# bluemoon-o2/walker-gym

Hardware: AMD Instinct MI355X
Metric: env-steps/sec (whole node) at 65 536 walkers; 1/2/4/8 MI355X scaling (higher is better)
Workload: dtype f32

## Files before the change

include/walker_hip.h:

```cpp
#ifndef WALKER_HIP_H
#define WALKER_HIP_H
#include <stdint.h>

#ifdef __cplusplus
extern "C" {
#endif

typedef struct ihipStream_t *hipStream_t;
typedef struct ihipEvent_t *hipEvent_t;

#define WG_ABI_VERSION 14
#define WG_EINVAL (-1)
#define WG_ERANGE (-2)
#define WG_EHIP (-3)

typedef struct wg_params {
    double g, dampk, ground, groundk, grounddamp, friction, dt;
    double pk, vk, ak, mk;
    int32_t in3d, max_steps;
    int32_t midform;
    int32_t conmid;
    int32_t spring_mode;
    int32_t action_mode;
    int32_t integrator;
    int32_t pair_mode;
    double pair_g;
    double pair_k;
    double pair_e;
    double bounce_k;
    double g3_gravity[3];
    double g3_damping;
    double g3_air;
    double g3_ground_level;
    double g3_restitution;
    double g3_friction;
    int32_t g3_ground;
    int32_t friction_mode;
} wg_params;

typedef struct wg_edge {
    uint32_t ij;
    float rest, k, c;
} wg_edge;

typedef struct wg_batch {
    int32_t N, M, K, A;
    int32_t ragged;
    const int32_t *mass_off, *edge_off, *muscle_off;
    float *pos, *vel, *acc;
    const float *mass;
    const wg_edge *edges;
    const uint16_t *inc;
    const uint16_t *inc_off;
    float *muscle_x;
    const float *muscle_bounds;
    const float *muscle_stride;
    int32_t *steps;
    uint8_t *contact;
    const uint8_t *pinned;
    const double *charge;
    double *radius;
    const int32_t *row;
    const uint8_t *bounce_set;
} wg_batch;

typedef struct wg_outputs {
    float *obs;       int32_t obs_stride;
    float *reward;    uint8_t *done;
    float *centroid;  float *energy;
    int64_t obs_step, out_step;
    int32_t obs_pad_clean;
    int32_t *steps;
    uint8_t *nonfinite;
    float *momentum;
} wg_outputs;

typedef struct wg_launch_info {
    int32_t threads, walkers_per_block, blocks, lds_bytes;
} wg_launch_info;

int wg_abi_version(void);
const char *wg_last_error(void);

int wg_step(const wg_batch *b, const wg_params *p, const float *action, int32_t action_cols,
            int32_t action_stride, int64_t action_step, const wg_outputs *o, int32_t n_steps,
            const int32_t *plan, int32_t plan_blocks, hipStream_t stream);

int wg_rollout(const wg_batch *b, const wg_params *p, const float *action, int32_t action_cols,
               int32_t action_stride, int64_t action_step, const wg_outputs *o, int32_t n_steps,
               const int32_t *plan, int32_t plan_blocks, hipStream_t stream);

typedef struct wg_range {
    const wg_batch *batch;
    const wg_outputs *outputs;
    int64_t action_offset;
    const int32_t *plan;
    int32_t plan_blocks;
    hipStream_t stream;
} wg_range;

int wg_step_ranges(const wg_range *ranges, int32_t n, const wg_params *p, const float *action, int32_t action_cols,
                   int32_t action_stride, hipEvent_t *events);

int wg_run_ranges(const wg_range *ranges, int32_t n, const wg_params *p, const float *action, int32_t action_cols,
                  int32_t action_stride, int64_t action_step, int32_t n_steps, hipEvent_t *events);

int wg_observe(const wg_batch *b, const wg_params *p, const wg_outputs *o, const int32_t *plan,
               int32_t plan_blocks, hipStream_t stream);

typedef wg_params wg_obs_cfg;
int wg_step_simple(const wg_batch *b, const float *action, const wg_params *p, int32_t n_steps, hipStream_t stream);
int wg_observe_simple(const wg_batch *b, const wg_obs_cfg *cfg, float *obs, float *reward, uint8_t *done,
                      float *centroid, float *energy, hipStream_t stream);

int wg_reset(const wg_batch *b, const wg_params *p, const float *noise, const uint8_t *mask,
             hipStream_t stream);

int wg_reset_noise(const wg_batch *b, const float *noise, hipStream_t stream);

int wg_plan_ragged(const int32_t *mass_off, const int32_t *edge_off, const int32_t *muscle_off,
                   int32_t N, int32_t *plan, int32_t max_blocks);

int wg_plan_waves(const int32_t *mass_off, const int32_t *edge_off, const int32_t *muscle_off,
                  int32_t N, int32_t *plan, int32_t max_tiles);
int wg_wave_edge_passes(int32_t M, int32_t K);

int wg_plan_errors(int32_t clear);

int wg_launch_geometry(const wg_batch *b, wg_launch_info *info);

int wg_debug_stamps(unsigned long long *host, int n);

int wg_launch_floor(int32_t mode, int32_t blocks, int32_t threads, const float *in, float *out, int32_t n_launches,
                    hipStream_t stream);

int wg_time_step(const wg_batch *batch, const wg_params *params, const float *action, int32_t action_cols,
                 int32_t action_stride, int64_t action_step, const wg_outputs *out, int32_t n_steps,
                 const int32_t *plan, int32_t plan_blocks, hipStream_t stream, float *ms_per_launch);

#ifdef __cplusplus
}
#endif
#endif
```

walker_gym_amd/_lib.py:

```python
from __future__ import annotations

import ctypes as C
import os
import threading

HERE = os.path.dirname(os.path.abspath(__file__))
LIB_NAME = "libwalker_hip.so"
LIB_PATH = os.path.join(HERE, LIB_NAME)
ABI_VERSION = 14

WG_EINVAL, WG_ERANGE, WG_EHIP = -1, -2, -3

_vp = C.c_void_p


class WgParams(C.Structure):
    _fields_ = [(n, C.c_double) for n in ("g", "dampk", "ground", "groundk", "grounddamp", "friction", "dt",
                                           "pk", "vk", "ak", "mk")] + \
               [(n, C.c_int32) for n in ("in3d", "max_steps", "midform", "conmid", "spring_mode", "action_mode",
                                         "integrator", "pair_mode")] + \
               [(n, C.c_double) for n in ("pair_g", "pair_k", "pair_e", "bounce_k")] + \
               [("g3_gravity", C.c_double * 3)] + \
               [(n, C.c_double) for n in ("g3_damping", "g3_air", "g3_ground_level", "g3_restitution",
                                          "g3_friction")] + [("g3_ground", C.c_int32), ("friction_mode", C.c_int32)]


class WgBatch(C.Structure):
    _fields_ = [("N", C.c_int32), ("M", C.c_int32), ("K", C.c_int32), ("A", C.c_int32),
                ("ragged", C.c_int32),
                ("mass_off", _vp), ("edge_off", _vp), ("muscle_off", _vp),
                ("pos", _vp), ("vel", _vp), ("acc", _vp), ("mass", _vp),
                ("edges", _vp),
                ("inc", _vp), ("inc_off", _vp),
                ("muscle_x", _vp), ("muscle_bounds", _vp), ("muscle_stride", _vp),
                ("steps", _vp), ("contact", _vp), ("pinned", _vp),
                ("charge", _vp), ("radius", _vp), ("row", _vp), ("bounce_set", _vp)]


class WgOutputs(C.Structure):
    _fields_ = [("obs", _vp), ("obs_stride", C.c_int32), ("reward", _vp), ("done", _vp),
                ("centroid", _vp), ("energy", _vp), ("obs_step", C.c_int64), ("out_step", C.c_int64),
                ("obs_pad_clean", C.c_int32), ("steps", _vp), ("nonfinite", _vp), ("momentum", _vp)]


class WgRange(C.Structure):
    _fields_ = [("batch", C.POINTER(WgBatch)), ("outputs", C.POINTER(WgOutputs)), ("action_offset", C.c_int64),
                ("plan", _vp), ("plan_blocks", C.c_int32), ("stream", _vp)]


class WgLaunchInfo(C.Structure):
    _fields_ = [("threads", C.c_int32), ("walkers_per_block", C.c_int32), ("blocks", C.c_int32),
                ("lds_bytes", C.c_int32)]


EXPORTS = ("wg_abi_version", "wg_last_error", "wg_step", "wg_step_ranges", "wg_run_ranges", "wg_rollout", "wg_observe",
           "wg_step_simple", "wg_observe_simple", "wg_reset", "wg_reset_noise", "wg_plan_ragged", "wg_plan_waves",
           "wg_wave_edge_passes", "wg_plan_errors", "wg_launch_geometry", "wg_launch_floor", "wg_time_step")

_lib = None
_lock = threading.Lock()


class WalkerHipError(RuntimeError):
    pass


def load(path: str | None = None):
    global _lib
    with _lock:
        if _lib is not None:
            return _lib
        p = path or os.environ.get("WALKER_HIP_LIB", LIB_PATH)
        if not os.path.exists(p):
            raise WalkerHipError(
                f"{p} not found: build it with `python -m walker_gym_amd.build` (hipcc --offload-arch=gfx950); "
                "walker_gym_amd has no CPU fallback")
        L = C.CDLL(p)
        L.wg_abi_version.restype = C.c_int
        L.wg_last_error.restype = C.c_char_p
        L.wg_step.argtypes = [C.POINTER(WgBatch), C.POINTER(WgParams), _vp, C.c_int32, C.c_int32, C.c_int64,
                              C.POINTER(WgOutputs), C.c_int32, _vp, C.c_int32, _vp]
        L.wg_rollout.argtypes = L.wg_step.argtypes
        L.wg_step_ranges.argtypes = [C.POINTER(WgRange), C.c_int32, C.POINTER(WgParams), _vp, C.c_int32, C.c_int32,
                                     C.POINTER(_vp)]
        L.wg_run_ranges.argtypes = [C.POINTER(WgRange), C.c_int32, C.POINTER(WgParams), _vp, C.c_int32, C.c_int32,
                                    C.c_int64, C.c_int32, C.POINTER(_vp)]
        L.wg_observe.argtypes = [C.POINTER(WgBatch), C.POINTER(WgParams), C.POINTER(WgOutputs), _vp, C.c_int32, _vp]
        L.wg_step_simple.argtypes = [C.POINTER(WgBatch), _vp, C.POINTER(WgParams), C.c_int32, _vp]
        L.wg_observe_simple.argtypes = [C.POINTER(WgBatch), C.POINTER(WgParams), _vp, _vp, _vp, _vp, _vp, _vp]
        L.wg_reset.argtypes = [C.POINTER(WgBatch), C.POINTER(WgParams), _vp, _vp, _vp]
        L.wg_reset_noise.argtypes = [C.POINTER(WgBatch), _vp, _vp]
        L.wg_plan_ragged.argtypes = [_vp, _vp, _vp, C.c_int32, _vp, C.c_int32]
        L.wg_plan_waves.argtypes = [_vp, _vp, _vp, C.c_int32, _vp, C.c_int32]
        L.wg_wave_edge_passes.argtypes = [C.c_int32, C.c_int32]
        L.wg_plan_errors.argtypes = [C.c_int32]
        L.wg_launch_geometry.argtypes = [C.POINTER(WgBatch), C.POINTER(WgLaunchInfo)]
        L.wg_launch_floor.argtypes = [C.c_int32, C.c_int32, C.c_int32, _vp, _vp, C.c_int32, _vp]
        L.wg_time_step.argtypes = L.wg_step.argtypes + [C.POINTER(C.c_float)]
        for f in EXPORTS[2:]:
            getattr(L, f).restype = C.c_int
        v = L.wg_abi_version()
        if v != ABI_VERSION:
            raise WalkerHipError(f"{p}: ABI version {v}, expected {ABI_VERSION}")
        _lib = L
        return L


def check(rc: int, what: str) -> int:
    if rc < 0:
        msg = load().wg_last_error().decode(errors="replace")
        exc = ValueError if rc in (WG_EINVAL, WG_ERANGE) else WalkerHipError
        raise exc(f"{what}: {msg} (code {rc})")
    return rc
```

walker_gym_amd/csrc/walker_hip.hip:

```cpp

#include <hip/hip_runtime.h>
#include <hip/hip_ext.h>

#include <algorithm>
#include <cstdarg>
#include <cstdint>
#include <cstdio>
#include <cstdlib>
#include <cstring>
#include <vector>

#include "walker_hip.h"
#include "powf2.h"

namespace {

thread_local char g_err[512] = "";

int fail(int code, const char *fmt, ...) __attribute__((format(printf, 2, 3)));
int fail(int code, const char *fmt, ...) {
    va_list ap;
    va_start(ap, fmt);
    vsnprintf(g_err, sizeof g_err, fmt, ap);
    va_end(ap);
    return code;
}

constexpr int WG_MAX_M = 1024;
constexpr double CONFIG_R = 16e-36;
constexpr int EPL = 4;
constexpr int NTHREADS = 256;
constexpr int MAXT = 512;
#ifndef WG_ABLATE
#define WG_ABLATE 0
#endif

struct KParams {
    float neg_g, neg_dampk, ground, neg_groundk, neg_grounddamp, friction, dt;
    float pk, vk, ak, mk, done_y;
    float dt2;
    double g;
    int max_steps, midform, conmid, spring_mode, action_mode;
    int integrator;
    int pair_mode;
    double pair_g, pair_k, pair_e;
    float bounce_kh;
    float g3g[3], g3_damp, g3_dragc, g3_level, g3_rest, g3_fric;
    int g3_ground;
    int friction_mode;
    int prio;
    int xcd;
};

struct KOut {
    float *obs, *reward;
    uint8_t *done;
    float *centroid, *energy;
    int32_t *steps;
    int64_t obs_step, out_step;
    int32_t obs_stride, obs_pad_clean;
};
inline KOut kout(const wg_outputs &o) {
    return KOut{o.obs, o.reward, o.done, o.centroid, o.energy, o.steps, o.obs_step, o.out_step, o.obs_stride,
                o.obs_pad_clean};
}

thread_local hipEvent_t g_kev_start = nullptr, g_kev_stop = nullptr;
#define WG_KLAUNCH(KERNEL, GRID, BLOCK, LDS, STREAM, ...)                                                          \
    do {                                                                                                          \
        if (g_kev_start)                                                                                          \
            hipExtLaunchKernelGGL(KERNEL, GRID, BLOCK, LDS, STREAM, g_kev_start, g_kev_stop, 0u, __VA_ARGS__);    \
        else                                                                                                      \
            hipLaunchKernelGGL(KERNEL, GRID, BLOCK, LDS, STREAM, __VA_ARGS__);                                    \
    } while (0)

__device__ __forceinline__ int xcd_block(int bid, int nwg) {
    const int q = nwg >> 3, r = nwg & 7, x = bid & 7;
    return (x < r ? x * (q + 1) : r * (q + 1) + (x - r) * q) + (bid >> 3);
}

struct Geo {
    int W, Pcap, Ecap, Ucap;
    int threads;
    int lds;
    float invM, invK, invA;
    int tbytes;
    int lite;
};

#ifdef WG_STAMPS
__device__ unsigned long long g_stamps[(1 << 16) * 8];
#define STAMP(k)                                                                                          \
    do {                                                                                                  \
        const unsigned long long t_ = __builtin_amdgcn_s_memtime();                                      \
        if ((threadIdx.x & 63) == 0 && stamp_wave < (1 << 16)) g_stamps[stamp_wave * 8 + (k)] = t_;      \
    } while (0)
#else
#define STAMP(k) do {} while (0)
#endif

struct Carve {
    double *t;
    float *pos, *vel, *acc, *m;
    float *df;
    uint32_t *inc;
    float *x;
    float *nrm, *ke, *pe;
    float *red;
    int *moff, *eoff, *uoff;
};

__host__ __device__ inline int align16(int b) { return (b + 15) & ~15; }

__device__ __forceinline__ int caller_row(const wg_batch &b, int w) { return b.row ? b.row[w] : w; }

enum { CV_T, CV_POS, CV_VEL, CV_ACC, CV_M, CV_DF, CV_INC, CV_X, CV_NRM, CV_KE, CV_PE, CV_RED,
       CV_MOFF, CV_EOFF, CV_UOFF, CV_N };
__host__ __device__ inline int carve_walk(const Geo &g, int *off) {
    int b = 0, k = 0;
    auto take = [&](int bytes) { off[k++] = b; b += align16(bytes); };
    const int full = g.lite ? 0 : 1;
    take(g.tbytes); take(g.Pcap * 12); take(g.Pcap * 12);
    take(full * g.Pcap * 12); take(full * g.Pcap * 4);
    take(g.Ecap * 12);
    take(g.Ecap * 4 + 16); take(g.Ucap * 4);
    take(full * g.Pcap * 4); take(full * g.Pcap * 4); take(full * g.Pcap * 4);
    take(full * g.W * 32);
    take(full * (g.W + 1) * 4); take(full * (g.W + 1) * 4); take(full * (g.W + 1) * 4);
    return b;
}
__host__ __device__ inline int carve_bytes(const Geo &g) { int off[CV_N]; return carve_walk(g, off); }
__device__ inline Carve carve(char *s, const Geo &g) {
    int o[CV_N];
    carve_walk(g, o);
    Carve c;
    c.t = reinterpret_cast<double *>(s + o[CV_T]); c.pos = reinterpret_cast<float *>(s + o[CV_POS]);
    c.vel = reinterpret_cast<float *>(s + o[CV_VEL]); c.acc = reinterpret_cast<float *>(s + o[CV_ACC]);
    c.m = reinterpret_cast<float *>(s + o[CV_M]); c.df = reinterpret_cast<float *>(s + o[CV_DF]);
    c.inc = reinterpret_cast<uint32_t *>(s + o[CV_INC]); c.x = reinterpret_cast<float *>(s + o[CV_X]);
    c.nrm = reinterpret_cast<float *>(s + o[CV_NRM]); c.ke = reinterpret_cast<float *>(s + o[CV_KE]);
    c.pe = reinterpret_cast<float *>(s + o[CV_PE]); c.red = reinterpret_cast<float *>(s + o[CV_RED]);
    c.moff = reinterpret_cast<int *>(s + o[CV_MOFF]); c.eoff = reinterpret_cast<int *>(s + o[CV_EOFF]);
    c.uoff = reinterpret_cast<int *>(s + o[CV_UOFF]);
    return c;
}

__device__ __forceinline__ float sqrt_mid(float s) {
    const float r = __builtin_amdgcn_sqrtf(s);
    const float rd = __uint_as_float(__float_as_uint(r) - 1u), ru = __uint_as_float(__float_as_uint(r) + 1u);
    float o = (__builtin_fmaf(-rd, r, s) <= 0.f) ? rd : r;
    return (__builtin_fmaf(-ru, r, s) > 0.f) ? ru : o;
}
__device__ inline float np_norm3(float x, float y, float z) {
    const float px = x * x, py = y * y, pz = z * z;
    double s = 0.0;
    s += (double)px; s += (double)py; s += (double)pz;
    return sqrtf((float)s);
}
__device__ inline float np_dot3(float ax, float ay, float az, float bx, float by, float bz) {
    const float p0 = ax * bx, p1 = ay * by, p2 = az * bz;
    double s = 0.0;
    s += (double)p0; s += (double)p1; s += (double)p2;
    return (float)s;
}
__device__ inline float seq_sum_lds(float r, const float *a, int n, int st) {
    int i = 0;
    for (; i + 4 <= n; i += 4) {
        const float x0 = a[i * st], x1 = a[(i + 1) * st], x2 = a[(i + 2) * st], x3 = a[(i + 3) * st];
        r = (((r + x0) + x1) + x2) + x3;
    }
    for (; i < n; i++) r += a[i * st];
    return r;
}
__device__ inline float pw_leaf(const float *a, int n, int st) {
    if (n < 8) return seq_sum_lds(0.f, a, n, st);
    float r0 = a[0], r1 = a[st], r2 = a[2 * st], r3 = a[3 * st];
    float r4 = a[4 * st], r5 = a[5 * st], r6 = a[6 * st], r7 = a[7 * st];
    int i = 8;
    for (; i < n - (n % 8); i += 8) {
        const float *p = a + i * st;
        r0 += p[0]; r1 += p[st]; r2 += p[2 * st]; r3 += p[3 * st];
        r4 += p[4 * st]; r5 += p[5 * st]; r6 += p[6 * st]; r7 += p[7 * st];
    }
    const float res = ((r0 + r1) + (r2 + r3)) + ((r4 + r5) + (r6 + r7));
    return seq_sum_lds(res, a + i * st, n - i, st);
}
__device__ inline void dual_sum_lds(const float *a, int sa, const float *p, int sp, int n, float &rs, float &rp) {
    float s = 0.f;
    int i = 0;
    if (n < 8) {
        float q = 0.f;
        for (; i + 4 <= n; i += 4) {
            const float x0 = a[i * sa], x1 = a[(i + 1) * sa], x2 = a[(i + 2) * sa], x3 = a[(i + 3) * sa];
            const float y0 = p[i * sp], y1 = p[(i + 1) * sp], y2 = p[(i + 2) * sp], y3 = p[(i + 3) * sp];
            s = (((s + x0) + x1) + x2) + x3;
            q = (((q + y0) + y1) + y2) + y3;
        }
        for (; i < n; i++) { s += a[i * sa]; q += p[i * sp]; }
        rs = s; rp = q;
        return;
    }
    float r0 = p[0], r1 = p[sp], r2 = p[2 * sp], r3 = p[3 * sp];
    float r4 = p[4 * sp], r5 = p[5 * sp], r6 = p[6 * sp], r7 = p[7 * sp];
    for (; i < 8; i += 4) {
        const float x0 = a[i * sa], x1 = a[(i + 1) * sa], x2 = a[(i + 2) * sa], x3 = a[(i + 3) * sa];
        s = (((s + x0) + x1) + x2) + x3;
    }
    for (; i < n - (n % 8); i += 8) {
        const float *q = p + i * sp, *b = a + i * sa;
        const float x0 = b[0], x1 = b[sa], x2 = b[2 * sa], x3 = b[3 * sa];
        const float x4 = b[4 * sa], x5 = b[5 * sa], x6 = b[6 * sa], x7 = b[7 * sa];
        r0 += q[0]; r1 += q[sp]; r2 += q[2 * sp]; r3 += q[3 * sp];
        r4 += q[4 * sp]; r5 += q[5 * sp]; r6 += q[6 * sp]; r7 += q[7 * sp];
        s = (((((((s + x0) + x1) + x2) + x3) + x4) + x5) + x6) + x7;
    }
    float res = ((r0 + r1) + (r2 + r3)) + ((r4 + r5) + (r6 + r7));
    for (; i < n; i++) { s += a[i * sa]; res += p[i * sp]; }
    rs = s; rp = res;
}
template <int D>
__device__ inline float pw_tree(const float *a, int n, int st) {
    if (D == 0 || n <= 128) return pw_leaf(a, n, st);
    int n2 = n / 2;
    n2 -= n2 % 8;
    return pw_tree<(D > 0 ? D - 1 : 0)>(a, n2, st) + pw_tree<(D > 0 ? D - 1 : 0)>(a + n2 * st, n - n2, st);
}
template <int PWD>
__device__ inline float np_pairwise(const float *a, int n, int st) { return pw_tree<PWD>(a, n, st); }

__device__ inline int locate(const int *off, int n, int x) {
    int lo = 0, hi = n - 1;
    while (lo < hi) {
        const int mid = (lo + hi + 1) >> 1;
        if (off[mid] <= x) lo = mid; else hi = mid - 1;
    }
    return lo;
}

__device__ inline int fdiv(int idx, int d, float inv) {
    (void)d;
    return (int)(((float)idx + 0.5f) * inv);
}

__device__ inline float fdiv_exact(float x, double y) { return (float)((double)x * y); }
constexpr int TINY_EXP = -79;
__device__ __forceinline__ int fexp(float x) { return __builtin_amdgcn_frexp_expf(x); }
__device__ __forceinline__ int fexp3(float a, float b, float c) { return min(min(fexp(a), fexp(b)), fexp(c)); }
__device__ __forceinline__ bool divisor_ok(float m) {
    const int e = fexp(m);
    return e >= -19 && e <= 21 && m != 0.f;
}
__device__ inline float fdiv_mk(float x, float m, float yf) {
    const float q = x * yf;
    if (!__builtin_isfinite(q) || yf == 0.f) return q;
    if (__builtin_expect(fexp(x) < TINY_EXP || !divisor_ok(m), 0)) return x / m;
    return __builtin_fmaf(__builtin_fmaf(-q, m, x), yf, q);
}
__device__ inline float fxsign(float v, uint32_t s) { return __uint_as_float(__float_as_uint(v) ^ s); }
__device__ inline double dxsign(double v, uint32_t s) {
    return __hiloint2double(__double2hiint(v) ^ (int)s, __double2loint(v));
}
__device__ inline double ddiv_fast(double a, double b, double y) {
    const double q = a * y;
    return __builtin_fma(__builtin_fma(-q, b, a), y, q);
}
__device__ inline float fdiv_fast(float x, float m, float yf) {
    const float q = x * yf;
    return __builtin_fmaf(__builtin_fmaf(-q, m, x), yf, q);
}
__device__ inline double ddiv_exact(double a, double b, double y) {
    const double q = a * y;
    if (!__builtin_isfinite(q) || y == 0.0) return q;
    return __builtin_fma(__builtin_fma(-q, b, a), y, q);
}
__device__ inline double ddiv_f32d(double a, double b, double y) {
    const double q = a * y;
    const double m = __builtin_fma(__builtin_fma(-q, b, a), y, q);
    const double am = __builtin_fabs(m);
    if (__builtin_expect(am >= 0x1p-800 && am <= 0x1p800, 1)) return m;
    return a == 0.0 ? q : a / b;
}

__device__ __forceinline__ double rcp64_nr(double d) {
    double y = __builtin_amdgcn_rcp(d);
    double e = __builtin_fma(-d, y, 1.0);
    y = __builtin_fma(y, e, y);
    e = __builtin_fma(-d, y, 1.0);
    return __builtin_fma(y, e, y);
}

__device__ __forceinline__ double rcp64_nr(double d);
__device__ __forceinline__ bool divisor_ok(float m);
__device__ __forceinline__ double recip_m(float mf) {
    const double md = (double)mf;
    double y = rcp64_nr(md);
    if (__builtin_expect(!divisor_ok(mf), 0)) y = 1.0 / md;
    return y;
}

__device__ __forceinline__ float fdiv_count(float x, float fM, double yM) {
    float q = (float)((double)x * yM);
    if (__builtin_expect(__builtin_fabsf(x) < 0x1p-100f, 0)) q = x / fM;
    return q;
}


__device__ __attribute__((noinline)) float np_sq_cold(float x) { return pw_pow2(x); }
template <bool INL = false>
__device__ __forceinline__ float np_sq(float x) {
    float f;
    if (__builtin_expect(!pw_pow2_fast(x, &f), 0)) f = INL ? pw_pow2(x) : np_sq_cold(x);
    return f;
}
__shared__ double s_pw_log2[32];
__shared__ unsigned long long s_pw_exp2[32];
__device__ __forceinline__ void pw_tables_to_lds(int tid) {
    if (tid < 32) { s_pw_log2[tid] = PW_LOG2_TAB[tid]; s_pw_exp2[tid] = PW_EXP2_TAB[tid]; }
}
__device__ __forceinline__ float pw_pow2_lds(float x) {
    unsigned int ix = pw_asu32(x) & 0x7fffffffu;
    if (ix == 0u || ix >= 0x7f800000u) return x * x;
    if (ix < 0x00800000u) {
        ix = pw_asu32(pw_asfloat(ix) * 0x1p23f) & 0x7fffffffu;
        ix -= 23u << 23;
    }
    const unsigned int tmp = ix - 0x3f330000u;
    const int i = (int)((tmp >> 19) & 15u);
    const unsigned int top = tmp & 0xff800000u;
    const int k = (int)top >> 23;
    const double invc = s_pw_log2[2 * i], logc = s_pw_log2[2 * i + 1];
    const double z = (double)pw_asfloat(ix - top);
    const double r = PW_FMA(z, invc, -1.0);
    const double y0 = logc + (double)k;
    const double r2 = r * r;
    double y = PW_FMA(0x1.27616c9496e0bp-2, r, -0x1.71969a075c67ap-2);
    const double p = PW_FMA(0x1.ec70a6ca7baddp-2, r, -0x1.7154748bef6c8p-1);
    const double r4 = r2 * r2;
    double q = PW_FMA(0x1.71547652ab82bp+0, r, y0);
    q = PW_FMA(p, r2, q);
    y = PW_FMA(y, r4, q);
    const double xd = 2.0 * y;
    if (((pw_asu64(xd) >> 47) & 0xffffu) >= (pw_asu64(126.0) >> 47)) {
        if (xd > 0x1.fffffffd1d571p+6) return pw_asfloat(0x7f800000u);
        if (xd <= -150.0) return 0.0f;
    }
    const double shift = 0x1.8p+47;
    double kd = xd + shift;
    const unsigned long long ki = pw_asu64(kd);
    kd -= shift;
    const double rr = xd - kd;
    const unsigned long long t = s_pw_exp2[ki & 31u] + (ki << 47);
    const double sc = pw_asdouble(t);
    const double zz = PW_FMA(0x1.c6af84b912394p-5, rr, 0x1.ebfce50fac4f3p-3);
    const double rr2 = rr * rr;
// ... 895 lines not shown
            if (pairs) {
                ax = s.acc[3 * lp]; ay = s.acc[3 * lp + 1]; az = s.acc[3 * lp + 2];
                mass_tail(kp, mf, (float)(1.0 / md), s.pos + 3 * lp, s.vel + 3 * lp, px, py, pz, vx, vy, vz, ax, ay,
                          az, hit, b.pinned && b.pinned[P0 + lp]);
            } else {
                mass_step(kp, s.t, s.df, s_inc16 + 2 * lb, lb, s0, (WG_ABLATE & 2) ? min(s1, s0 + 1) : s1, mf,
                          s.pos + 3 * lp, s.vel + 3 * lp, px, py, pz, vx, vy, vz, ax, ay, az, hit, kp.spring_mode,
                          b.pinned && b.pinned[P0 + lp], tiny_blk);
            }
            if (b.contact) b.contact[P0 + lp] = (uint8_t)hit;
            if (b.radius) b.radius[P0 + lp] = hit ? 3.0 : 1.0;
            s.pos[3 * lp] = px; s.pos[3 * lp + 1] = py; s.pos[3 * lp + 2] = pz;
            s.vel[3 * lp] = vx; s.vel[3 * lp + 1] = vy; s.vel[3 * lp + 2] = vz;
            if (SHFL) {
                float *ga = b.acc + 3 * ((size_t)P0 + lp);
                ga[0] = ax; ga[1] = ay; ga[2] = az;
            } else {
                s.acc[3 * lp] = ax; s.acc[3 * lp + 1] = ay; s.acc[3 * lp + 2] = az;
            }
            nv = np_norm3(vx, vy, vz);
            ke = mf * np_sq_t<true>(nv);
            pe = (float)(md * kp.g) * (py - kp.ground);
            if (!SHFL) { s.nrm[lp] = nv; s.ke[lp] = ke; s.pe[lp] = pe; }
        }
    } else {
        for (int lp = tid; lp < nP; lp += T) {
            const float mf = SHFL ? my_m : s.m[lp];
            vx = s.vel[3 * lp]; vy = s.vel[3 * lp + 1]; vz = s.vel[3 * lp + 2];
            px = s.pos[3 * lp]; py = s.pos[3 * lp + 1]; pz = s.pos[3 * lp + 2];
            if (SHFL) {
                const float *ga = b.acc + 3 * ((size_t)P0 + lp);
                ax = ga[0]; ay = ga[1]; az = ga[2];
            } else {
                ax = s.acc[3 * lp]; ay = s.acc[3 * lp + 1]; az = s.acc[3 * lp + 2];
            }
            nv = np_norm3(vx, vy, vz);
            ke = mf * np_sq_t<true>(nv);
            pe = (float)((double)mf * kp.g) * (py - kp.ground);
            if (!SHFL) { s.nrm[lp] = nv; s.ke[lp] = ke; s.pe[lp] = pe; }
        }
    }

    float midx = 0.f, midy = 0.f, midz = 0.f;
    float sumx = 0.f, sumy = 0.f, sumz = 0.f;
    const bool is_mass = tid < nP;
    const int my_q = tid - my_lm;
    if (SHFL) {
        const int M = b.M;
        const int gbase = (tid & ~63) + ((lane / M) * M);
        float sx, sy, sz;
        seq_sum3_lanes(px, py, pz, gbase, M, sx, sy, sz);
        const float ysum = pw_sum_lanes(py, gbase, M, lane), vsum = pw_sum_lanes(nv, gbase, M, lane);
        const float ksum = pw_sum_lanes(ke, gbase, M, lane), psum = pw_sum_lanes(pe, gbase, M, lane);
        const unsigned long long gmask = (M == 64) ? ~0ull : (((1ull << M) - 1ull) << (gbase & 63));
        const unsigned long long hb = __ballot(is_mass && (py - kp.ground < 0.f));
        const unsigned long long sb = __ballot(is_mass && nv < 0.1f);
        const int hits = __popcll(hb & gmask);
        const bool all_stopped = (sb & gmask) == gmask;
        const float fM = (float)M;
        midx = sx / fM; midy = sy / fM; midz = sz / fM;
        sumx = sx; sumy = sy; sumz = sz;
        if (is_mass && my_q == 0) {
            const size_t wg = (size_t)(w0 + my_wl);
            int steps = wsteps;
            if (STEP) { steps += 1; b.steps[wg] = steps; }
            if (o.steps) o.steps[wg] = steps;
            const float cy = ysum / fM;
            if (o.reward) {
                const float vpen = (-(vsum / fM)) * 0.1f;
                o.reward[wg] = (cy + vpen) + (float)(-(double)hits * 0.5);
            }
            if (o.done) {
                int done = steps >= kp.max_steps;
                if (!done && cy < kp.done_y) done = 1;
                if (!done && steps > 100) done = all_stopped;
                o.done[wg] = (uint8_t)done;
            }
            if (o.centroid) { o.centroid[3 * wg] = midx; o.centroid[3 * wg + 1] = midy; o.centroid[3 * wg + 2] = midz; }
            if (o.energy) o.energy[wg] = 0.5f * ksum + psum;
        }
    }
    __syncthreads();

    if (STEP) {
        stage_out(b.pos + 3 * (size_t)P0, s.pos, 3 * nP, tid, T);
        stage_out(b.vel + 3 * (size_t)P0, s.vel, 3 * nP, tid, T);
        if (!SHFL) stage_out(b.acc + 3 * (size_t)P0, s.acc, 3 * nP, tid, T);
    }
    if (!SHFL) {
        for (int idx = tid; idx < ((WG_ABLATE & 8) ? 0 : nw * 8); idx += T) {
            const int wl = idx >> 3, r = idx & 7;
            const int lm = RAGGED ? s.moff[wl] : wl * b.M;
            const int M = RAGGED ? s.moff[wl + 1] - lm : b.M;
            float v;
            if (r == 7) {
                int hits = 0, all = 1;
                for (int q = 0; q < M; q++) {
                    hits += (s.pos[3 * (lm + q) + 1] - kp.ground < 0.f);
                    all &= (s.nrm[lm + q] < 0.1f);
                }
                v = __int_as_float((hits << 1) | all);
            } else {
                const float *src = r < 3 ? s.pos + 3 * lm + r
                                 : r == 3 ? s.pos + 3 * lm + 1
                                 : r == 4 ? s.nrm + lm : r == 5 ? s.ke + lm : s.pe + lm;
                const int st = r <= 3 ? 3 : 1;
                if (r < 3) {
                    v = seq_sum_lds(0.f, src, M, st);
                } else {
                    v = np_pairwise<PWD>(src, M, st);
                }
            }
            s.red[idx] = v;
        }
        __syncthreads();
        if (tid < nw) {
            const int wl = tid;
            const int lm = RAGGED ? s.moff[wl] : wl * b.M;
            const int M = RAGGED ? s.moff[wl + 1] - lm : b.M;
            const size_t ws = (size_t)(w0 + wl);
            const size_t wg = (size_t)caller_row(b, w0 + wl);
            const float fM = (float)M;
            const float *rd = s.red + 8 * wl;
            const float cy = rd[3] / fM;
            const int packed = __float_as_int(rd[7]);
            const int hits = packed >> 1, all = packed & 1;
            int steps = wsteps;
            if (STEP) { steps += 1; b.steps[ws] = steps; }
            if (o.steps) o.steps[wg] = steps;
            if (o.reward) {
                const float av = rd[4] / fM;
                const float vpen = (-av) * 0.1f;
                const float cpen = (float)(-(double)hits * 0.5);
                o.reward[wg] = (cy + vpen) + cpen;
            }
            if (o.done) {
                int done = steps >= kp.max_steps;
                if (!done && cy < kp.done_y) done = 1;
                if (!done && steps > 100) done = all;
                o.done[wg] = (uint8_t)done;
            }
            if (o.centroid) {
                o.centroid[3 * wg] = rd[0] / fM; o.centroid[3 * wg + 1] = rd[1] / fM; o.centroid[3 * wg + 2] = rd[2] / fM;
            }
            if (o.energy) o.energy[wg] = 0.5f * rd[5] + rd[6];
        }
    }

    if (o.obs && !(WG_ABLATE & 16)) {
        constexpr int d = IN3D ? 3 : 2, per = 3 * d;
        const int stride = o.obs_stride;
        float *ob = o.obs + (uint32_t)w0 * (uint32_t)stride;
        float *tile = RAGGED ? nullptr : reinterpret_cast<float *>(s.t);
        const int nmid = kp.conmid ? 3 : 0;
        if (SHFL) {
            if (is_mass) {
                float *row = tile + (size_t)my_wl * stride + per * my_q;
                const float pm[3] = {px, py, pz}, vm[3] = {vx, vy, vz}, am[3] = {ax, ay, az};
                const float mm[3] = {kp.midform == 2 ? sumx : midx, kp.midform == 2 ? sumy : midy,
                                     kp.midform == 2 ? sumz : midz};
#pragma unroll
                for (int c = 0; c < d; c++) {
                    row[c] = kp.midform ? (pm[c] - mm[c]) * kp.pk : pm[c] * kp.pk;
                    row[d + c] = vm[c] * kp.vk;
                    row[2 * d + c] = am[c] * kp.ak;
                }
                if (my_q == 0 && nmid) {
                    float *wrow = tile + (size_t)my_wl * stride + per * b.M;
                    wrow[0] = kp.midform ? mm[0] : 0.f; wrow[1] = kp.midform ? mm[1] : 0.f; wrow[2] = kp.midform ? mm[2] : 0.f;
                }
                if (my_q == 0)
                    for (int r = per * b.M + nmid + b.A; r < stride; r++) tile[(size_t)my_wl * stride + r] = 0.f;
            }
        } else {
            for (int lp = tid; lp < nP; lp += T) {
                int wl, lm;
                if (lp == tid) { wl = my_wl; lm = my_lm; }
                else if (RAGGED) { wl = locate(s.moff, nw, lp); lm = s.moff[wl]; }
                else { wl = fdiv(lp, b.M, geo.invM); lm = wl * b.M; }
                const int M = RAGGED ? s.moff[wl + 1] - lm : b.M;
                const float fM = (float)M;
                float *row = (RAGGED ? o.obs + (size_t)caller_row(b, w0 + wl) * stride : tile + (size_t)wl * stride) +
                             per * (lp - lm);
#pragma unroll
                for (int c = 0; c < d; c++) {
                    const float pv = s.pos[3 * lp + c];
                    const float mid = kp.midform == 2 ? s.red[8 * wl + c] : s.red[8 * wl + c] / fM;
                    row[c] = kp.midform ? (pv - mid) * kp.pk : pv * kp.pk;
                    row[d + c] = s.vel[3 * lp + c] * kp.vk;
                    row[2 * d + c] = s.acc[3 * lp + c] * kp.ak;
                }
            }
            for (int wl = tid; wl < nw; wl += T) {
                const int lm = RAGGED ? s.moff[wl] : wl * b.M;
                const int M = RAGGED ? s.moff[wl + 1] - lm : b.M;
                const int A = RAGGED ? s.uoff[wl + 1] - s.uoff[wl] : b.A;
                float *row = RAGGED ? o.obs + (size_t)caller_row(b, w0 + wl) * stride : tile + (size_t)wl * stride;
                if (nmid)
                    for (int c = 0; c < 3; c++)
                        row[per * M + c] = kp.midform == 2 ? s.red[8 * wl + c] : kp.midform ? s.red[8 * wl + c] / (float)M : 0.f;
                for (int r = per * M + nmid + A; r < stride; r++) row[r] = 0.f;
            }
        }
        for (int u = tid; u < nU; u += T) {
            int wl, ua, M;
            if (RAGGED) { wl = locate(s.uoff, nw, u); ua = u - s.uoff[wl]; M = s.moff[wl + 1] - s.moff[wl]; }
            else { wl = fdiv(u, b.A, geo.invA); ua = u - wl * b.A; M = b.M; }
            (RAGGED ? o.obs + (size_t)caller_row(b, w0 + wl) * stride : tile + (size_t)wl * stride)[per * M + nmid + ua] =
                s.x[u] * kp.mk;
        }
        if (!RAGGED) {
            __syncthreads();
            stage_out(ob, tile, nw * stride, tid, T);
        }
    }
}


struct LeanGeo {
    int wpw;
    int wpb;
    int lgM;
    int slice;
    int off_df, off_inc, off_x;
    int pl;
    float invK, invA, invM;
    int nblk;
};

__device__ __forceinline__ void wave_sync() {
    __builtin_amdgcn_fence(__ATOMIC_RELEASE, "wavefront");
    __builtin_amdgcn_wave_barrier();
    __builtin_amdgcn_fence(__ATOMIC_ACQUIRE, "wavefront");
}


__device__ __forceinline__ float lane_gather(float v, int src_byte) {
    return __int_as_float(__builtin_amdgcn_ds_bpermute(src_byte, __float_as_int(v)));
}

__device__ __forceinline__ void spring_terms_cold(const EdgeRec &e, float x, float r0, float r1, float r2, double &t0,
                                               double &t1, double &t2, float &d0, float &d1, float &d2,
                                               int spring_mode) {
    const float cur = np_norm3(-r0, -r1, -r2);
    const float dx = cur - x;
    double dist = (double)cur;
    if (CONFIG_R > dist) dist = CONFIG_R;
    const float fsz = (spring_mode == 1 || !(dx < 0.f && edge_string(e.ij))) ? (-dx) * e.k : 0.f;
    const float nf = -fsz;
    d0 = r0; d1 = r1; d2 = r2;
    if (cur > 0.f) { d0 = r0 / cur; d1 = r1 / cur; d2 = r2 / cur; }
    if (spring_mode == 1) {
        t0 = (double)(fsz * d0); t1 = (double)(fsz * d1); t2 = (double)(fsz * d2);
    } else {
        t0 = (double)(nf * r0) / dist; t1 = (double)(nf * r1) / dist; t2 = (double)(nf * r2) / dist;
    }
}


__device__ __forceinline__ void spring_terms(const EdgeRec &e, float x, float pix, float piy, float piz, float pjx,
                                             float pjy, float pjz, float vix, float viy, float viz, float vjx,
                                             float vjy, float vjz, double &t0, double &t1, double &t2, float &g0,
                                             float &g1, float &g2, int spring_mode, bool pos_ok) {
    const float r0 = pjx - pix, r1 = pjy - piy, r2 = pjz - piz;
    float d0, d1, d2;
    const float sq = (float)(((double)(r0 * r0) + (double)(r1 * r1)) + (double)(r2 * r2));
    const bool mid = sq >= 0x1p-40f && sq < 0x1p40f;
    const float cur = sqrt_mid(sq);
    const float dx = cur - x;
    const double dist = (double)cur;
    const double yc = rcp64_nr(dist);
    const float fsz = (spring_mode == 1 || !(dx < 0.f && edge_string(e.ij))) ? (-dx) * e.k : 0.f;
    const float nf = -fsz;
    const float ycf = (float)yc;
    d0 = fdiv_fast(r0, cur, ycf); d1 = fdiv_fast(r1, cur, ycf); d2 = fdiv_fast(r2, cur, ycf);
    if (spring_mode == 1) {
        t0 = (double)(fsz * d0); t1 = (double)(fsz * d1); t2 = (double)(fsz * d2);
    } else {
        t0 = ddiv_fast((double)(nf * r0), dist, yc);
        t1 = ddiv_fast((double)(nf * r1), dist, yc);
        t2 = ddiv_fast((double)(nf * r2), dist, yc);
    }
    bool rok = true;
    if (__builtin_expect(!pos_ok, 0)) rok = fexp3(r0, r1, r2) >= TINY_EXP;
    const bool fast_ok = mid && rok && __builtin_fabsf(nf) < 0x1p100f;
    if (__builtin_expect(!fast_ok, 0)) spring_terms_cold(e, x, r0, r1, r2, t0, t1, t2, d0, d1, d2, spring_mode);
    const float dk = np_dot3(vix - vjx, viy - vjy, viz - vjz, d0, d1, d2);
    const float dkc = dk * e.c;
    g0 = dkc * d0; g1 = dkc * d1; g2 = dkc * d2;
}
template <class TS>
__device__ __forceinline__ void spring_edge_regs(const EdgeRec &e, int le, float x, float pix, float piy, float piz,
                                                 float pjx, float pjy, float pjz, float vix, float viy, float viz,
                                                 float vjx, float vjy, float vjz, const TS &ts, int spring_mode, bool &gt,
                                                 bool pos_ok) {
    double t0, t1, t2;
    float g0, g1, g2;
    spring_terms(e, x, pix, piy, piz, pjx, pjy, pjz, vix, viy, viz, vjx, vjy, vjz, t0, t1, t2, g0, g1, g2, spring_mode,
                 pos_ok);
    ts.put(le, t0, t1, t2, g0, g1, g2);
    gt = gt || fexp3(g0, g1, g2) < TINY_EXP;
}

template <int NE>
struct LeanIn {
    float p3[3], v3[3];
    EdgeRec er[NE];
    uint32_t gi[NE];
    float mf;
    int io0, io1, wsteps, pin;
    float x, lo, hi, stp, a;
};

struct LeanTile {
    int w0, nw, nP, nE, nU, wl, q, mu_wl, mu_ua;
    uint32_t P0, E0, U0;
    bool is_mass, is_mus, acts;
};

__device__ __forceinline__ LeanTile lean_tile_of(const wg_batch &b, const float *action, int action_cols,
                                                 const LeanGeo &lg, int tile, int lane) {
    LeanTile t;
    t.w0 = tile * lg.wpw;
    t.nw = min(lg.wpw, b.N - t.w0);
    t.nP = t.nw * b.M; t.nE = t.nw * b.K; t.nU = t.nw * b.A;
    t.P0 = (uint32_t)t.w0 * b.M; t.E0 = (uint32_t)t.w0 * b.K; t.U0 = (uint32_t)t.w0 * b.A;
    t.wl = lane >> lg.lgM; t.q = lane & (b.M - 1);
    t.is_mass = lane < t.nP;
    t.is_mus = lane < t.nU;
    t.mu_wl = b.A > 0 ? fdiv(lane, b.A, lg.invA) : 0;
    t.mu_ua = lane - t.mu_wl * b.A;
    t.acts = action != nullptr && t.is_mus && t.mu_ua < action_cols;
    return t;
}

template <typename T>
__device__ __forceinline__ const T &at_u32(const T *base, uint32_t byte_off) {
    return *reinterpret_cast<const T *>(reinterpret_cast<const char *>(base) + (size_t)byte_off);
}
template <typename T>
__device__ __forceinline__ T &at_u32w(T *base, uint32_t byte_off) {
    return *reinterpret_cast<T *>(reinterpret_cast<char *>(base) + (size_t)byte_off);
}
#define WG_ST(base, e, n) (&at_u32w((base), (uint32_t)(n) * 4u * (uint32_t)(e)))
__device__ __forceinline__ float neg_half_count(int n) { return -0.5f * (float)n; }
template <int NE>
__device__ __forceinline__ void lean_load_mass(const wg_batch &b, const LeanTile &t, int lane, LeanIn<NE> &L) {
    L.mf = 0.f; L.io0 = 0; L.io1 = 0; L.wsteps = 0; L.pin = 0;
    const int ln = min(lane, t.nP - 1);
    const int wl = ln >> (31 - __builtin_clz(b.M)), q = ln & (b.M - 1);
    L.mf = at_u32(b.mass, 4u * (t.P0 + ln));
    if (b.pinned) L.pin = at_u32(b.pinned, t.P0 + ln);
    const uint32_t io = (uint32_t)(t.w0 + wl) * (b.M + 1) + q;
    L.io0 = at_u32(b.inc_off, 2u * io); L.io1 = at_u32(b.inc_off, 2u * io + 2u);
    L.wsteps = at_u32(b.steps, 4u * (uint32_t)(t.w0 + wl));
}
template <int NE>
__device__ __forceinline__ void lean_load_muscles(const wg_batch &b, const KParams &kp, const float *__restrict__ action,
                                                  int action_stride, const LeanTile &t, int lane, LeanIn<NE> &L) {
    L.x = 0.f; L.lo = 0.f; L.hi = 0.f; L.stp = 0.f; L.a = 0.f;
    if (t.nU > 0) {
        const uint32_t ul = t.U0 + min(lane, t.nU - 1);
        L.x = at_u32(b.muscle_x, 4u * ul);
        if (action && action_stride > 0) {
            const float2 bd = at_u32(reinterpret_cast<const float2 *>(b.muscle_bounds), 8u * ul);
            L.lo = bd.x; L.hi = bd.y;
            if (kp.action_mode == 1) L.stp = at_u32(b.muscle_stride, 4u * ul);
            const int wl = min(t.mu_wl, t.nw - 1), ua = max(0, min(t.mu_ua, action_stride - 1));
            L.a = at_u32(action, 4u * ((uint32_t)(t.w0 + wl) * (uint32_t)action_stride + (uint32_t)ua));
        }
    }
}
template <int NE>
__device__ __forceinline__ void lean_load(const wg_batch &b, const KParams &kp, const float *__restrict__ action,
                                          int action_stride, const LeanTile &t, int lane, LeanIn<NE> &L) {
    const uint32_t pl = t.P0 + min(lane, t.nP - 1);
    const float *gp = &at_u32(b.pos, 12u * pl), *gv = &at_u32(b.vel, 12u * pl);
    L.p3[0] = gp[0]; L.p3[1] = gp[1]; L.p3[2] = gp[2];
    L.v3[0] = gv[0]; L.v3[1] = gv[1]; L.v3[2] = gv[2];
#pragma unroll
    for (int it = 0; it < NE; it++) {
        const uint32_t le = t.E0 + (uint32_t)min(lane + 64 * it, t.nE - 1);
        const uint4 v = at_u32(reinterpret_cast<const uint4 *>(b.edges), 16u * le);
        L.er[it] = EdgeRec{v.x, __uint_as_float(v.y), __uint_as_float(v.z), __uint_as_float(v.w)};
        L.gi[it] = at_u32(reinterpret_cast<const uint32_t *>(b.inc), 4u * le);
    }
    lean_load_mass<NE>(b, t, lane, L);
    lean_load_muscles<NE>(b, kp, action, action_stride, t, lane, L);
    if (!t.is_mass) {
        L.p3[0] = 0.f; L.p3[1] = 0.f; L.p3[2] = 0.f; L.v3[0] = 0.f; L.v3[1] = 0.f; L.v3[2] = 0.f;
        L.mf = 0.f; L.pin = 0; L.io0 = 0; L.io1 = 0;
    }
    if (!t.is_mus) { L.x = 0.f; L.lo = 0.f; L.hi = 0.f; L.stp = 0.f; }
    if (!t.acts) L.a = 0.f;
}

__device__ __forceinline__ double lane_gather_d(double v, int src_byte) {
    return __hiloint2double(__builtin_amdgcn_ds_bpermute(src_byte, __double2hiint(v)),
                            __builtin_amdgcn_ds_bpermute(src_byte, __double2loint(v)));
}

__device__ __forceinline__ float pw_pow2_lanes(float x, double tl, double te) {
    unsigned int ix = pw_asu32(x) & 0x7fffffffu;
    const bool special = ix == 0u || ix >= 0x7f800000u;
    if (ix < 0x00800000u && ix != 0u) {
        ix = pw_asu32(pw_asfloat(ix) * 0x1p23f) & 0x7fffffffu;
        ix -= 23u << 23;
    }
    const unsigned int tmp = ix - 0x3f330000u;
    const int i = (int)((tmp >> 19) & 15u);
    const unsigned int top = tmp & 0xff800000u;
    const int k = (int)top >> 23;
    const double invc = lane_gather_d(tl, (2 * i) << 2), logc = lane_gather_d(tl, (2 * i + 1) << 2);
    const double z = (double)pw_asfloat(ix - top);
    const double r = PW_FMA(z, invc, -1.0);
    const double y0 = logc + (double)k;
    const double r2 = r * r;
    double y = PW_FMA(0x1.27616c9496e0bp-2, r, -0x1.71969a075c67ap-2);
    const double p = PW_FMA(0x1.ec70a6ca7baddp-2, r, -0x1.7154748bef6c8p-1);
    const double r4 = r2 * r2;
    double q = PW_FMA(0x1.71547652ab82bp+0, r, y0);
    q = PW_FMA(p, r2, q);
    y = PW_FMA(y, r4, q);
    const double xd = 2.0 * y;
    const bool big = ((pw_asu64(xd) >> 47) & 0xffffu) >= (pw_asu64(126.0) >> 47);
    const double shift = 0x1.8p+47;
    double kd = xd + shift;
    const unsigned long long ki = pw_asu64(kd);
    kd -= shift;
    const double rr = xd - kd;
    const unsigned long long t = pw_asu64(lane_gather_d(te, (int)(ki & 31u) << 2)) + (ki << 47);
    const double sc = pw_asdouble(t);
    const double zz = PW_FMA(0x1.c6af84b912394p-5, rr, 0x1.ebfce50fac4f3p-3);
    const double rr2 = rr * rr;
    double yy = PW_FMA(0x1.62e42ff0c52d6p-1, rr, 1.0);
    yy = PW_FMA(zz, rr2, yy);
    float res = (float)(yy * sc);
    if (big && xd > 0x1.fffffffd1d571p+6) res = pw_asfloat(0x7f800000u);
    else if (big && xd <= -150.0) res = 0.0f;
    return special ? x * x : res;
}
__device__ __forceinline__ float np_sq_wave(float x, double tl, double te) {
    float f;
    const bool need = !pw_pow2_fast(x, &f);
    if (__builtin_expect(__ballot(need) != 0ull, 0)) {
        const float g = pw_pow2_lanes(x, tl, te);
        if (need) f = g;
    }
    return f;
}

__device__ __forceinline__ void pair_central(double coef, double sq, const float *p3, float mf, int lane, int M,
                                             bool is_mass, float &ax, float &ay, float &az, bool self_first = false) {
    const int gb = lane & ~(M - 1), q = lane & (M - 1);
    const double md = (double)mf, ym = 1.0 / md;
    const float sx = ax, sy = ay, sz = az;
    bool bad = false;
    {
        for (int pj = 0; pj < M; pj++) {
            const int src = (gb + pj) << 2;
            const float ox = lane_gather(p3[0], src), oy = lane_gather(p3[1], src), oz = lane_gather(p3[2], src);
            const double os = lane_gather_d(sq, src);
            if (!is_mass || pj == q) continue;
            const float d0 = ox - p3[0], d1 = oy - p3[1], d2 = oz - p3[2];
            const bool lo = pj < q && !self_first;
            pair_central_fast(coef, lo ? os : sq, lo ? sq : os, d0, d1, d2, md, ym, ax, ay, az, bad);
        }
        bad = is_mass && (bad || !__builtin_isfinite(ax + ay + az));
    }
    if (__builtin_expect(__ballot(bad) != 0, 0)) {
        float cx = sx, cy = sy, cz = sz;
        for (int pj = 0; pj < M; pj++) {
            const int src = (gb + pj) << 2;
            const float ox = lane_gather(p3[0], src), oy = lane_gather(p3[1], src), oz = lane_gather(p3[2], src);
            const double os = lane_gather_d(sq, src);
            if (!bad || pj == q) continue;
            const float d0 = ox - p3[0], d1 = oy - p3[1], d2 = oz - p3[2];
            const bool lo = pj < q && !self_first;
            pair_central_term(coef, lo ? os : sq, lo ? sq : os, d0, d1, d2, md, ym, cx, cy, cz);
        }
        if (bad) { ax = cx; ay = cy; az = cz; }
    }
}

__device__ __forceinline__ void pair_bounce(float kh, double rs, int bs, const float *p3, float mf, int lane, int M,
                                            bool is_mass, float &ax, float &ay, float &az) {
    const int gb = lane & ~(M - 1), q = lane & (M - 1);
    const double md = (double)mf, ym = 1.0 / md;
    for (int ph = 0; ph < 3; ph++) {
        for (int pj = 0; pj < M; pj++) {
            const int src = (gb + pj) << 2;
            const float ox = lane_gather(p3[0], src), oy = lane_gather(p3[1], src), oz = lane_gather(p3[2], src);
            const double orad = lane_gather_d(rs, src);
            const int obs = __builtin_amdgcn_ds_bpermute(src, bs);
            const bool on = ph == 1 ? pj != q && (bs & 1) && (obs & 2)
                                    : (ph == 0 ? pj < q : pj > q) && (obs & 1) && (bs & 2);
            if (!is_mass || !on) continue;
            const float d0 = ox - p3[0], d1 = oy - p3[1], d2 = oz - p3[2];
            const float cur = np_norm3(d0, d1, d2);
            const double x = rs + orad;
            if (!((double)cur <= x)) continue;
            const float dx = cur - (float)x;
            const float nf = -((-dx) * kh);
            bounce_term(cur, nf, d0, d1, d2, md, ym, ax, ay, az);
        }
    }
}

__device__ __forceinline__ void pair_g2_gravity(double g, const float *p3, float mf, int lane, int M, bool is_mass,
                                                float &ax, float &ay, float &az) {
    const int gb = lane & ~(M - 1), q = lane & (M - 1);
    const double md = (double)mf, ym = 1.0 / md;
    ax = 0.f; ay = 0.f; az = 0.f;
    for (int pj = 0; pj < M; pj++) {
        const int src = (gb + pj) << 2;
        const float ox = lane_gather(p3[0], src), oy = lane_gather(p3[1], src), oz = lane_gather(p3[2], src);
        const float om = lane_gather(mf, src);
        if (!is_mass || pj == q) continue;
        const double mo = (double)om;
        g2_gravity_term(((-g) * (pj < q ? mo : md)) * (pj < q ? md : mo), ox - p3[0], oy - p3[1], oz - p3[2], mf, ym,
                        ax, ay, az);
    }
}

__device__ __forceinline__ void pair_forces(const wg_batch &b, const KParams &kp, const float *p3, float mf,
                                         uint32_t pl, int lane, int M, bool is_mass, float &ax, float &ay,
                                         float &az) {
    if (kp.pair_mode & 1) pair_central(kp.pair_g, (double)mf, p3, mf, lane, M, is_mass, ax, ay, az);
    if (kp.pair_mode & 2) {
        const double e = (b.charge && is_mass) ? b.charge[pl] : kp.pair_e;
        pair_central(kp.pair_k, e, p3, mf, lane, M, is_mass, ax, ay, az);
    }
    if (kp.pair_mode & 4) {
        const double rs = is_mass ? b.radius[pl] : 0.0;
        const int bs = b.bounce_set ? (is_mass ? (int)b.bounce_set[pl] : 0) : 3;
        pair_bounce(kp.bounce_kh, rs, bs, p3, mf, lane, M, is_mass, ax, ay, az);
    }
    if (kp.pair_mode & 8) pair_g2_gravity(kp.pair_g, p3, mf, lane, M, is_mass, ax, ay, az);
    if (kp.pair_mode & 16) {
        const double e = (b.charge && is_mass) ? b.charge[pl] : kp.pair_e;
        pair_central(kp.pair_k, e, p3, mf, lane, M, is_mass, ax, ay, az, true);
    }
}



typedef TermsAoS LeanTerms;
__device__ __forceinline__ LeanTerms lean_terms(char *sl, const LeanGeo &lg) {
    return TermsAoS{reinterpret_cast<double *>(sl), reinterpret_cast<float *>(sl + lg.off_df)};
}

template <bool IN3D, int NE, bool RES = false>
__device__ __forceinline__ void lean_compute(const wg_batch &b, const KParams &kp, const KOut &o,
                                             const LeanGeo &lg, char *sl, const LeanTile &t, int lane,
                                             LeanIn<NE> &L, bool last = true) {
    const bool store = !RES || last;
    const int M = b.M, K = b.K, A = b.A;
    const int w0 = t.w0, nE = t.nE;
    const int wl = t.wl, q = t.q, mu_wl = t.mu_wl, mu_ua = t.mu_ua;
    const bool is_mass = t.is_mass, is_mus = t.is_mus, acts = t.acts;
    const uint32_t pl = t.P0 + lane, ul = t.U0 + lane;
    const LeanTerms ts = lean_terms(sl, lg);
#ifdef WG_STAMPS
    const int stamp_wave = t.w0 / lg.wpw;
#endif
    uint32_t *s_inc = reinterpret_cast<uint32_t *>(sl + lg.off_inc);
    float *s_x = reinterpret_cast<float *>(sl + lg.off_x);
    const float mf = L.mf;
    const bool pin = L.pin != 0;
    double sq_tl = 0.0, sq_te = 0.0;
    if (NE == 1 && !RES) {
        sq_tl = PW_LOG2_TAB[lane & 31];
        sq_te = pw_asdouble(PW_EXP2_TAB[lane & 31]);
    }

    if (!RES) {
#pragma unroll
        for (int it = 0; it < NE; it++)
            if (lane + 64 * it < nE) s_inc[lane + 64 * it] = L.gi[it];
        if (lane == 0) s_inc[nE] = 0u;
    }
    float x = L.x;
    if (acts) {
        x = (kp.action_mode == 1) ? ((L.a != 0.f) ? x + L.stp : x - L.stp) : x + L.a;
        if (L.lo > x) x = L.lo;
        if (L.hi < x) x = L.hi;
        if (store) *WG_ST(b.muscle_x, ul, 1) = x;
    }
    if (is_mus) s_x[lane] = x;
    double ym = recip_m(mf);
    if (!RES) asm volatile("" : "+v"(ym));
    wave_sync();
    STAMP(2);

    bool dead = false;
    if ((!RES || NE == 1) && kp.pair_mode == 0) {
        const bool nanp = is_mass && (__builtin_isnan(L.p3[0]) || __builtin_isnan(L.p3[1]) || __builtin_isnan(L.p3[2]));
        if (__builtin_expect(__ballot(nanp) != 0ull, 0)) {
            const unsigned long long db = __ballot(nanp && !pin && L.io1 > L.io0);
            const unsigned long long gm = (M == 64) ? ~0ull : (((1ull << M) - 1ull) << (lane & ~(M - 1)));
            dead = is_mass && (db & gm) == gm;
            if (dead) {
                L.p3[0] = (float)q; L.p3[1] = 0.f; L.p3[2] = 0.f;
                L.v3[0] = 0.f; L.v3[1] = 0.f; L.v3[2] = 0.f;
            }
        }
    }

    bool gtiny = false;
    const bool pos_ok = __all(fexp3(L.p3[0], L.p3[1], L.p3[2]) >= -55);
    struct Gath { float v[12]; };
    auto gather = [&](int it, Gath &g) {
        const int le = lane + 64 * it;
        const int ewl = fdiv(le, K, lg.invK);
        const uint32_t ij = L.er[it].ij;
        const int bi = ((ewl << lg.lgM) + edge_i(ij)) << 2, bj = ((ewl << lg.lgM) + edge_j(ij)) << 2;
#pragma unroll
        for (int c = 0; c < 3; c++) {
            if (WG_ABLATE & 512) {
                g.v[c] = L.p3[c]; g.v[3 + c] = L.p3[c] + (float)(bj - bi); g.v[6 + c] = L.v3[c]; g.v[9 + c] = L.v3[c];
                continue;
            }
            g.v[c] = lane_gather(L.p3[c], bi); g.v[3 + c] = lane_gather(L.p3[c], bj);
            g.v[6 + c] = lane_gather(L.v3[c], bi); g.v[9 + c] = lane_gather(L.v3[c], bj);
        }
    };
    auto spring = [&](int it, const Gath &g) {
        const int le = lane + 64 * it;
        const EdgeRec e = L.er[it];
        const int ewl = fdiv(le, K, lg.invK), ew = le - (int)__umul24(ewl, K);
        const bool mus = le < nE && ew < A;
        const float xs = s_x[mus ? (int)__umul24(ewl, A) + ew : 0];
        const float xr = mus ? xs : e.rest;
        if (le < nE) {
            if (WG_ABLATE & 1) {
                ts.put(le, xr + g.v[0] + g.v[3] + g.v[6] + g.v[9], g.v[1] + g.v[4] + g.v[7] + g.v[10],
                       g.v[2] + g.v[5] + g.v[8] + g.v[11], e.k, e.c, 0.f);
            } else {
                spring_edge_regs(e, le, xr, g.v[0], g.v[1], g.v[2], g.v[3], g.v[4], g.v[5], g.v[6], g.v[7], g.v[8],
                                 g.v[9], g.v[10], g.v[11], ts, 0, gtiny, pos_ok);
            }
        }
    };
#pragma unroll
    for (int it = 0; it < NE; it++) {
        if (64 * it >= nE) continue;
        if ((WG_ABLATE & 4096) && it == NE - 1 && it > 0) {
            const int le = lane + 64 * it;
            if (le < nE) ts.put(le, 0.0, 0.0, 0.0, 0.f, 0.f, 0.f);
            continue;
        }
        Gath g;
        gather(it, g);
        spring(it, g);
    }
    wave_sync();
    const bool wave_tiny = __any(gtiny);
    STAMP(3);

    EnvTerms et{};
    if (!RES) et = env_terms(kp, mf, (float)ym, L.v3[0], L.v3[1], L.v3[2]);
    float px = 0.f, py = 0.f, pz = 0.f, vx = 0.f, vy = 0.f, vz = 0.f, ax = 0.f, ay = 0.f, az = 0.f;
    float nv = 0.f, ke = 0.f, pe = 0.f;
    bool hit = false;
    if (is_mass) {
        const int r1 = (WG_ABLATE & 2) ? min(L.io1, L.io0 + 1) : L.io1;
        const int lb = wl * K;
        if (!RES)
            mass_accumulate_v2(ts, reinterpret_cast<const uint16_t *>(s_inc) + 2 * lb, lb, L.io0, r1, mf, ym, ax, ay, az,
                               wave_tiny);
        else
            mass_accumulate<LeanTerms, !RES>(ts, reinterpret_cast<const uint16_t *>(s_inc) + 2 * lb, lb, L.io0, r1, mf,
                                             ax, ay, az, 0, wave_tiny);
    }
    if (!RES && kp.pair_mode) pair_forces(b, kp, L.p3, mf, pl, lane, M, is_mass, ax, ay, az);
    if (is_mass) {
        mass_tail(kp, mf, (float)ym, L.p3, L.v3, px, py, pz, vx, vy, vz, ax, ay, az, hit, pin,
                  !RES ? &et : nullptr);
        if (dead) {
            px = __builtin_nanf(""); py = px; pz = px; vx = px; vy = px; vz = px; ax = px; ay = px; az = px;
            hit = false;
        }
        if (b.radius && store) b.radius[pl] = hit ? 3.0 : 1.0;
        nv = np_norm3(vx, vy, vz);
        if (!(NE == 1 && !RES)) ke = dead ? nv : mf * np_sq<NE == 1>(nv);
        pe = (float)((double)mf * kp.g) * (py - kp.ground);
    }
    if (NE == 1 && !RES) {
        const float sq = np_sq_wave(dead ? 0.f : nv, sq_tl, sq_te);
        if (is_mass) ke = dead ? nv : mf * sq;
    }
    STAMP(4);

    const int gbase = lane & ~(M - 1);
    const WalkerSums ws = (WG_ABLATE & 4) ? WalkerSums{px, py, pz, py, nv, ke, pe}
                                          : walker_sums(px, py, pz, nv, ke, pe, gbase, M, lane);
    const float sx = ws.sx, sy = ws.sy, sz = ws.sz, ysum = ws.ysum, vsum = ws.vsum, ksum = ws.ksum, psum = ws.psum;
    const unsigned long long gmask = (M == 64) ? ~0ull : (((1ull << M) - 1ull) << gbase);
    const unsigned long long hb = __ballot(is_mass && (py - kp.ground < 0.f));
    const unsigned long long sb = __ballot(is_mass && nv < 0.1f);
    const float midx = sx * lg.invM, midy = sy * lg.invM, midz = sz * lg.invM;
    if (is_mass) {
        if (store) {
            float *gpo = WG_ST(b.pos, pl, 3), *gvo = WG_ST(b.vel, pl, 3), *gao = WG_ST(b.acc, pl, 3);
            gpo[0] = px; gpo[1] = py; gpo[2] = pz;
            gvo[0] = vx; gvo[1] = vy; gvo[2] = vz;
            gao[0] = ax; gao[1] = ay; gao[2] = az;
            if (b.contact) at_u32w(b.contact, pl) = (uint8_t)hit;
        }
        if (q == 0) {
            const uint32_t wg = (uint32_t)(w0 + wl);
            const int steps = L.wsteps + 1;
            if (store) *WG_ST(b.steps, wg, 1) = steps;
            if (RES) L.wsteps = steps;
            if (o.steps) *WG_ST(o.steps, wg, 1) = steps;
            const float cy = ysum * lg.invM;
            if (o.reward) {
                const float vpen = (-(vsum * lg.invM)) * 0.1f;
                *WG_ST(o.reward, wg, 1) = (cy + vpen) + neg_half_count((int)__popcll(hb & gmask));
            }
            if (o.done) {
                int done = steps >= kp.max_steps;
                if (!done && cy < kp.done_y) done = 1;
                if (!done && steps > 100) done = (sb & gmask) == gmask;
                at_u32w(o.done, wg) = (uint8_t)done;
            }
            if (o.centroid) {
                float *c = WG_ST(o.centroid, wg, 3);
                c[0] = midx; c[1] = midy; c[2] = midz;
            }
            if (o.energy) *WG_ST(o.energy, wg, 1) = 0.5f * ksum + psum;
        }
    }

    STAMP(5);
    if (o.obs && !(WG_ABLATE & 16)) {
        constexpr int d = IN3D ? 3 : 2, per = 3 * d;
        const int stride = o.obs_stride, nmid = kp.conmid ? 3 : 0;
        typedef float fvd __attribute__((ext_vector_type(d), aligned(4)));
        if (is_mass) {
            const uint32_t row0 = (uint32_t)(w0 + wl) * (uint32_t)stride;
            const float mm[3] = {kp.midform == 2 ? sx : midx, kp.midform == 2 ? sy : midy, kp.midform == 2 ? sz : midz};
            const float pm[3] = {px, py, pz}, vm[3] = {vx, vy, vz}, am[3] = {ax, ay, az};
            fvd vp, vv, va;
#pragma unroll
            for (int c = 0; c < d; c++) {
                vp[c] = kp.midform ? (pm[c] - mm[c]) * kp.pk : pm[c] * kp.pk;
                vv[c] = vm[c] * kp.vk;
                va[c] = am[c] * kp.ak;
            }
            float *dst = WG_ST(o.obs, row0 + per * q, 1);
            *reinterpret_cast<fvd *>(dst) = vp;
            *reinterpret_cast<fvd *>(dst + d) = vv;
            *reinterpret_cast<fvd *>(dst + 2 * d) = va;
            if (q == 0) {
                if (nmid) {
                    float *mrow = WG_ST(o.obs, row0 + per * M, 1);
                    mrow[0] = kp.midform ? mm[0] : 0.f; mrow[1] = kp.midform ? mm[1] : 0.f;
                    mrow[2] = kp.midform ? mm[2] : 0.f;
                }
                for (int r = per * M + nmid + A; r < stride; r++) *WG_ST(o.obs, row0 + r, 1) = 0.f;
            }
        }
        if (is_mus) *WG_ST(o.obs, (uint32_t)(w0 + mu_wl) * (uint32_t)stride + per * M + nmid + mu_ua, 1) = x * kp.mk;
    }
    if (RES) {
        L.p3[0] = px; L.p3[1] = py; L.p3[2] = pz;
        L.v3[0] = vx; L.v3[1] = vy; L.v3[2] = vz;
        L.x = x;
    }
    STAMP(6);
#ifdef WG_STAMPS
    if (lane == 0 && stamp_wave < (1 << 16)) {
        const unsigned hw = __builtin_amdgcn_s_getreg((31 << 11) | 4);
        const unsigned xcc = __builtin_amdgcn_s_getreg((31 << 11) | 20);
        g_stamps[stamp_wave * 8 + 7] = (unsigned long long)hw | ((unsigned long long)xcc << 32);
    }
#endif
}

constexpr int lean_waves(int NE) { return NE >= 8 ? 4 : 6; }

template <bool IN3D, int NE>
__global__ __launch_bounds__(256) __attribute__((amdgpu_waves_per_eu(lean_waves(NE)))) void walker_step_lean(
    wg_batch b, KParams kp, const float *__restrict__ action, int action_cols, int action_stride, KOut o,
    LeanGeo lg) {
    extern __shared__ __attribute__((aligned(16))) char smem[];
    const int lane = threadIdx.x & 63, wv = __builtin_amdgcn_readfirstlane(threadIdx.x >> 6);
    const int blk = (kp.xcd & 2) ? xcd_block(blockIdx.x, gridDim.x) : (int)blockIdx.x;
    const int tile = blk * lg.wpb + wv;
    if (tile * lg.wpw >= b.N) return;
#ifdef WG_STAMPS
    const int stamp_wave = tile;
#endif
    STAMP(0);
    const LeanTile t = lean_tile_of(b, action, action_cols, lg, tile, lane);
    LeanIn<NE> L;
    if (kp.prio) __builtin_amdgcn_s_setprio(2);
    lean_load<NE>(b, kp, action, action_stride, t, lane, L);
    if (kp.prio) __builtin_amdgcn_s_setprio(0);
    STAMP(1);
    lean_compute<IN3D, NE>(b, kp, o, lg, smem + wv * lg.slice, t, lane, L);
}

template <bool IN3D>
__global__ __launch_bounds__(256) __attribute__((amdgpu_waves_per_eu(lean_waves(1)))) void walker_step_lean1(
    float *pos, float *vel, const wg_edge *edges, const uint16_t *inc, int N, int M, int K, int wpw, int wpb, int nblkx,
    wg_batch b, KParams kp, const float *__restrict__ action, int action_cols, int action_stride, KOut o, LeanGeo lg) {
    extern __shared__ __attribute__((aligned(16))) char smem[];
    b.pos = pos; b.vel = vel; b.edges = edges; b.inc = inc; b.N = N; b.M = M; b.K = K;
    lg.nblk = nblkx & 0x3fffffff; lg.wpw = wpw; lg.wpb = wpb;
    kp.prio = (int)((unsigned)nblkx >> 31);
    const int lane = threadIdx.x & 63, wv = __builtin_amdgcn_readfirstlane(threadIdx.x >> 6);
    const int bid = blockIdx.x, xb = xcd_block(bid, lg.nblk);
    const int blk = (nblkx & 0x40000000) ? xb : bid;
    const int tile = blk * lg.wpb + wv;
    if (tile * lg.wpw >= b.N) return;
#ifdef WG_STAMPS
    const int stamp_wave = tile;
#endif
    STAMP(0);
    const LeanTile t = lean_tile_of(b, action, action_cols, lg, tile, lane);
    LeanIn<1> L;
    if (kp.prio) __builtin_amdgcn_s_setprio(2);
    lean_load<1>(b, kp, action, action_stride, t, lane, L);
    if (kp.prio) __builtin_amdgcn_s_setprio(0);
    STAMP(1);
    lean_compute<IN3D, 1>(b, kp, o, lg, smem + wv * lg.slice, t, lane, L);
}

template <bool IN3D, int NE>
__global__ __launch_bounds__(256) __attribute__((amdgpu_waves_per_eu(NE >= 8 ? 4 : 5))) void walker_rollout_lean(
    wg_batch b, KParams kp, const float *__restrict__ action, int action_cols, int action_stride, int64_t action_step,
    KOut o, int n_steps, LeanGeo lg) {
    extern __shared__ __attribute__((aligned(16))) char smem[];
    const int lane = threadIdx.x & 63, wv = __builtin_amdgcn_readfirstlane(threadIdx.x >> 6);
    const int tile = blockIdx.x * lg.wpb + wv;
    if (tile * lg.wpw >= b.N) return;
#ifdef WG_STAMPS
    const int stamp_wave = tile;
#endif
    const LeanTile t = lean_tile_of(b, action, action_cols, lg, tile, lane);
    LeanIn<NE> L;
    if (kp.prio) __builtin_amdgcn_s_setprio(2);
    lean_load<NE>(b, kp, action, action_stride, t, lane, L);
    if (kp.prio) __builtin_amdgcn_s_setprio(0);
    {
        uint32_t *s_inc = reinterpret_cast<uint32_t *>(smem + wv * lg.slice + lg.off_inc);
#pragma unroll
        for (int it = 0; it < NE; it++)
            if (lane + 64 * it < t.nE) s_inc[lane + 64 * it] = L.gi[it];
    }
#pragma clang loop unroll(disable)
    for (int s = 0; s < n_steps; s++) {
        int ln = lane;
        asm volatile("" : "+v"(ln));
        const LeanTile ts = lean_tile_of(b, action, action_cols, lg, tile, ln);
        float a_next = 0.f;
        if (ts.acts && s + 1 < n_steps)
            a_next = action[(size_t)(s + 1) * (size_t)action_step +
                            (size_t)(uint32_t)(ts.w0 + ts.mu_wl) * (uint32_t)action_stride + (uint32_t)ts.mu_ua];
        KOut os = o;
        if (os.obs) os.obs += (size_t)s * os.obs_step;
        if (os.reward) os.reward += (size_t)s * os.out_step;
        if (os.done) os.done += (size_t)s * os.out_step;
        if (os.energy) os.energy += (size_t)s * os.out_step;
        if (os.centroid) os.centroid += 3 * (size_t)s * os.out_step;
        if (os.steps) os.steps += (size_t)s * os.out_step;
        asm volatile("" : "+v"(L.mf), "+v"(L.io0), "+v"(L.io1), "+v"(L.lo), "+v"(L.hi), "+v"(L.stp));
#pragma unroll
        for (int it = 0; it < NE; it++) asm volatile("" : "+v"(L.er[it].ij), "+v"(L.er[it].rest), "+v"(L.er[it].k),
                                                     "+v"(L.er[it].c));
        lean_compute<IN3D, NE, true>(b, kp, os, lg, smem + wv * lg.slice, ts, ln, L, s == n_steps - 1);
        L.a = a_next;
        wave_sync();
    }
}

constexpr int RW_MAXW = 32;
__device__ int g_plan_error;

struct RagGeo {
    int wpb;
    int slice;
    int off_df, off_inc, off_x, off_wo;
};


template <bool IN3D, int NE>
__global__ __launch_bounds__(256) __attribute__((amdgpu_waves_per_eu(NE >= 8 ? 4 : NE >= 4 ? 5 : 6))) void walker_step_waves(
    wg_batch b, KParams kp, const float *__restrict__ action, int action_cols, int action_stride, KOut o,
    const int32_t *__restrict__ plan, int ntiles, RagGeo rg) {
    extern __shared__ __attribute__((aligned(16))) char smem[];
    const int lane = threadIdx.x & 63, wv = __builtin_amdgcn_readfirstlane(threadIdx.x >> 6);
    const int blk = (kp.xcd & 1) ? xcd_block(blockIdx.x, gridDim.x) : (int)blockIdx.x;
    const int tile = blk * rg.wpb + wv;
    if (tile >= ntiles) return;
#ifdef WG_STAMPS
    const int stamp_wave = tile;
#endif
    STAMP(0);
    char *sl = smem + wv * rg.slice;
    const TermsAoS ts{reinterpret_cast<double *>(sl), reinterpret_cast<float *>(sl + rg.off_df)};
    uint32_t *s_inc = reinterpret_cast<uint32_t *>(sl + rg.off_inc);
    float *s_x = reinterpret_cast<float *>(sl + rg.off_x);
    int *s_mo = reinterpret_cast<int *>(sl + rg.off_wo);
    int *s_eo = s_mo + (RW_MAXW + 1), *s_uo = s_eo + (RW_MAXW + 1), *s_row = s_uo + (RW_MAXW + 1);
    float *s_mid = reinterpret_cast<float *>(s_row + RW_MAXW);
    float *s_tp = reinterpret_cast<float *>(sl);
    float *s_tn = s_tp + 192, *s_tk = s_tn + 64, *s_te = s_tk + 64;
    float *s_red = reinterpret_cast<float *>(sl + rg.off_df);

    if (kp.prio) __builtin_amdgcn_s_setprio(2);
    const int w0 = plan[tile], w1 = plan[tile + 1], nw = w1 - w0;
    const int P0 = b.mass_off[w0], E0 = b.edge_off[w0], U0 = b.muscle_off[w0];
    const int nP = b.mass_off[w1] - P0, nE = b.edge_off[w1] - E0, nU = b.muscle_off[w1] - U0;
    if (nw < 1 || nw > RW_MAXW || nP < 1 || nP > 64 || nU > 64 || nE > 64 * NE) {
        if (lane == 0) atomicOr(&g_plan_error, 1);
        return;
    }
    const bool is_mass = lane < nP, is_mus = lane < nU;
    const int lw = min(lane, nw), lr = min(lane, nw - 1);
    int wmo = at_u32(b.mass_off, 4u * (w0 + lw)) - P0, weo = at_u32(b.edge_off, 4u * (w0 + lw)) - E0;
    int wuo = at_u32(b.muscle_off, 4u * (w0 + lw)) - U0;
    int wsteps = at_u32(b.steps, 4u * (w0 + lr));
    const int lp = P0 + min(lane, max(nP, 1) - 1);
    float p3[3], v3[3];
    {
        const float *gp = &at_u32(b.pos, 12u * lp), *gv = &at_u32(b.vel, 12u * lp);
        p3[0] = gp[0]; p3[1] = gp[1]; p3[2] = gp[2];
        v3[0] = gv[0]; v3[1] = gv[1]; v3[2] = gv[2];
    }
    float mf = at_u32(b.mass, 4u * lp);
    EdgeRec er[NE];
    uint32_t gi[NE];
    if (nE > 0) {
#pragma unroll
        for (int it = 0; it < NE; it++) {
            const uint32_t le = E0 + min(lane + 64 * it, nE - 1);
            const uint4 v = at_u32(reinterpret_cast<const uint4 *>(b.edges), 16u * le);
            er[it] = EdgeRec{v.x, __uint_as_float(v.y), __uint_as_float(v.z), __uint_as_float(v.w)};
            gi[it] = at_u32(reinterpret_cast<const uint32_t *>(b.inc), 4u * le);
        }
    }
    float mx = 0.f, mlo = 0.f, mhi = 0.f, mst = 0.f;
    if (nU > 0) {
        const uint32_t lu = U0 + min(lane, nU - 1);
        mx = at_u32(b.muscle_x, 4u * lu);
        if (action) {
            const float2 bd = at_u32(reinterpret_cast<const float2 *>(b.muscle_bounds), 8u * lu);
            mlo = bd.x; mhi = bd.y;
            if (kp.action_mode == 1) mst = at_u32(b.muscle_stride, 4u * lu);
        }
    }
    int wrow = w0 + lr, pin = 0;
    if (b.row && !(WG_ABLATE & 2048)) wrow = at_u32(b.row, 4u * (w0 + lr));
    if (b.pinned) pin = at_u32(b.pinned, (uint32_t)lp);
    if (lane <= nw) { s_mo[lane] = wmo; s_eo[lane] = weo; s_uo[lane] = wuo; }
    if (lane < nw) s_row[lane] = wrow;
    int mw = 0, uw = 0, eww[NE];
#pragma unroll
    for (int it = 0; it < NE; it++) eww[it] = 0;
    for (int w = 1; w < nw; w++) {
        const int so = __builtin_amdgcn_readlane(wmo, w), se = __builtin_amdgcn_readlane(weo, w);
        const int su = __builtin_amdgcn_readlane(wuo, w);
        mw += lane >= so;
        uw += lane >= su;
#pragma unroll
        for (int it = 0; it < NE; it++) eww[it] += lane + 64 * it >= se;
    }
    if (!is_mass) mw = 0;
    if (!is_mus) uw = 0;
    wave_sync();
    const int mlm = s_mo[mw], mlb = s_eo[mw];
    const uint32_t io = (uint32_t)lp + (uint32_t)(w0 + mw);
    int io0 = at_u32(b.inc_off, 2u * io), io1 = at_u32(b.inc_off, 2u * io + 2u);
    const int ua = lane - s_uo[uw];
    const bool acts = action != nullptr && is_mus && ua < action_cols;
    float act = 0.f;
    if (action && action_cols > 0)
        act = at_u32(action, 4u * ((uint32_t)s_row[uw] * (uint32_t)action_stride + (uint32_t)min(max(ua, 0), action_cols - 1)));
    if (!is_mass) {
        p3[0] = 0.f; p3[1] = 0.f; p3[2] = 0.f; v3[0] = 0.f; v3[1] = 0.f; v3[2] = 0.f;
        mf = 0.f; pin = 0; io0 = 0; io1 = 0;
    }
    if (!is_mus) { mx = 0.f; mlo = 0.f; mhi = 0.f; mst = 0.f; }
    if (!acts) act = 0.f;
    bool dead = false;
    {
        const bool nanp = is_mass && (__builtin_isnan(p3[0]) || __builtin_isnan(p3[1]) || __builtin_isnan(p3[2]));
        if (__builtin_expect(__ballot(nanp) != 0ull, 0)) {
            const unsigned long long db = __ballot(nanp && pin == 0 && io1 > io0);
            const int mwn = s_mo[mw + 1] - mlm;
            const unsigned long long gm = (mwn >= 64) ? ~0ull : (((1ull << mwn) - 1ull) << mlm);
            dead = is_mass && (db & gm) == gm;
            if (dead) {
                p3[0] = (float)(lane - mlm); p3[1] = 0.f; p3[2] = 0.f;
                v3[0] = 0.f; v3[1] = 0.f; v3[2] = 0.f;
            }
        }
    }
    if (kp.prio) __builtin_amdgcn_s_setprio(0);
    STAMP(1);

#pragma unroll
    for (int it = 0; it < NE; it++)
        if (lane + 64 * it < nE) s_inc[lane + 64 * it] = gi[it];
    if (lane == 0) s_inc[nE] = 0u;
    float x = mx;
    if (acts) {
        x = (kp.action_mode == 1) ? ((act != 0.f) ? x + mst : x - mst) : x + act;
        if (mlo > x) x = mlo;
        if (mhi < x) x = mhi;
        *WG_ST(b.muscle_x, U0 + lane, 1) = x;
    }
    if (is_mus) s_x[lane] = x;
    double ym = recip_m(mf);
    asm volatile("" : "+v"(ym));
    wave_sync();
    STAMP(2);

    bool gtiny = false;
    const bool pos_ok = __all(fexp3(p3[0], p3[1], p3[2]) >= -55);
#pragma unroll
    for (int it = 0; it < NE; it++) {
        if (64 * it >= nE) continue;
        const int le = lane + 64 * it;
        const EdgeRec e = er[it];
        const int ew_w = le < nE ? eww[it] : 0;
        const int elm = s_mo[ew_w], ew = le - s_eo[ew_w], eA = s_uo[ew_w + 1] - s_uo[ew_w];
        const int bi = (elm + edge_i(e.ij)) << 2, bj = (elm + edge_j(e.ij)) << 2;
        const float pix = lane_gather(p3[0], bi), piy = lane_gather(p3[1], bi), piz = lane_gather(p3[2], bi);
        const float pjx = lane_gather(p3[0], bj), pjy = lane_gather(p3[1], bj), pjz = lane_gather(p3[2], bj);
        const float vix = lane_gather(v3[0], bi), viy = lane_gather(v3[1], bi), viz = lane_gather(v3[2], bi);
        const float vjx = lane_gather(v3[0], bj), vjy = lane_gather(v3[1], bj), vjz = lane_gather(v3[2], bj);
        const bool mus = le < nE && ew < eA;
        const float xs = s_x[mus ? s_uo[ew_w] + ew : 0];
        const float xr = mus ? xs : e.rest;
        if (le < nE) {
            if (WG_ABLATE & 1)
                ts.put(le, xr + pix + pjx + vix + vjx, piy + pjy + viy + vjy, piz + pjz + viz + vjz, e.k, e.c, 0.f);
            else
                spring_edge_regs(e, le, xr, pix, piy, piz, pjx, pjy, pjz, vix, viy, viz, vjx, vjy, vjz, ts, 0, gtiny,
                                 pos_ok);
        }
    }
    wave_sync();
    const bool wave_tiny = __any(gtiny);
    STAMP(3);

    EnvTerms et{};
    et = env_terms(kp, mf, (float)ym, v3[0], v3[1], v3[2]);
    float px = 0.f, py = 0.f, pz = 0.f, vx = 0.f, vy = 0.f, vz = 0.f, ax = 0.f, ay = 0.f, az = 0.f;
    bool hit = false;
    if (is_mass) {
        mass_accumulate_v2(ts, reinterpret_cast<const uint16_t *>(s_inc) + 2 * mlb, mlb, io0,
                           (WG_ABLATE & 2) ? min(io1, io0 + 1) : io1, mf, ym, ax, ay, az, wave_tiny);
        mass_tail(kp, mf, (float)ym, p3, v3, px, py, pz, vx, vy, vz, ax, ay, az, hit, pin != 0, &et);
        if (dead) {
            px = __builtin_nanf(""); py = px; pz = px; vx = px; vy = px; vz = px; ax = px; ay = px; az = px;
            hit = false;
        }
        const uint32_t pl = (uint32_t)(P0 + lane);
        float *gpo = WG_ST(b.pos, pl, 3), *gvo = WG_ST(b.vel, pl, 3), *gao = WG_ST(b.acc, pl, 3);
        gpo[0] = px; gpo[1] = py; gpo[2] = pz;
        gvo[0] = vx; gvo[1] = vy; gvo[2] = vz;
        gao[0] = ax; gao[1] = ay; gao[2] = az;
        if (b.contact) at_u32w(b.contact, pl) = (uint8_t)hit;
        if (b.radius) b.radius[pl] = hit ? 3.0 : 1.0;
    }
    STAMP(4);
    const float nvm = is_mass ? np_norm3(vx, vy, vz) : 0.f;
    const unsigned long long hb = __ballot(is_mass && (py - kp.ground < 0.f));
    const unsigned long long sb = __ballot(is_mass && nvm < 0.1f);
    wave_sync();
    if (is_mass) {
        const float nv = nvm;
        s_tp[3 * lane] = px; s_tp[3 * lane + 1] = py; s_tp[3 * lane + 2] = pz;
        s_tn[lane] = nv;
        s_tk[lane] = dead ? nv : mf * np_sq(nv);
        s_te[lane] = (float)((double)mf * kp.g) * (py - kp.ground);
    }
    wave_sync();

    for (int idx = lane; idx < ((WG_ABLATE & 32) ? 0 : nw * 8); idx += 64) {
        const int w = idx >> 3, r = idx & 7;
        const int lm = s_mo[w], M = s_mo[w + 1] - lm;
        float v;
        if (r == 7) {
            const unsigned long long wm = (M == 64) ? ~0ull : (((1ull << M) - 1ull) << lm);
            v = __int_as_float((__popcll(hb & wm) << 1) | ((sb & wm) == wm ? 1 : 0));
        } else {
            const float *src = r == 3 ? s_tp + 3 * lm + 1 : r == 5 ? s_tk + lm : r == 6 ? s_te + lm : s_tn + lm;
            float vs, vp;
            dual_sum_lds(s_tp + 3 * lm + (r < 3 ? r : 0), 3, src, r == 3 ? 3 : 1, M, vs, vp);
            v = r < 3 ? vs : vp;
        }
        s_red[idx] = v;
    }
    wave_sync();
    if (lane < nw) {
        const int M = s_mo[lane + 1] - s_mo[lane];
        const float fM = (float)M;
        const double yM = rcp64_nr((double)M);
        const float *rd = s_red + 8 * lane;
        const float cy = fdiv_count(rd[3], fM, yM);
        const int packed = __float_as_int(rd[7]);
        const int hits = packed >> 1, all = packed & 1;
        const int steps = wsteps + 1;
        *WG_ST(b.steps, w0 + lane, 1) = steps;
        if (o.steps) *WG_ST(o.steps, wrow, 1) = steps;
        if (o.reward) *WG_ST(o.reward, wrow, 1) = (cy + (-fdiv_count(rd[4], fM, yM)) * 0.1f) + neg_half_count(hits);
        if (o.done) {
            int done = steps >= kp.max_steps;
            if (!done && cy < kp.done_y) done = 1;
            if (!done && steps > 100) done = all;
            at_u32w(o.done, (uint32_t)wrow) = (uint8_t)done;
        }
        const float mx = fdiv_count(rd[0], fM, yM), my = fdiv_count(rd[1], fM, yM), mz = fdiv_count(rd[2], fM, yM);
        s_mid[3 * lane] = mx; s_mid[3 * lane + 1] = my; s_mid[3 * lane + 2] = mz;
        if (o.centroid) {
            float *c = WG_ST(o.centroid, wrow, 3);
            c[0] = mx; c[1] = my; c[2] = mz;
        }
        if (o.energy) *WG_ST(o.energy, wrow, 1) = 0.5f * rd[5] + rd[6];
    }
    wave_sync();
    STAMP(5);

    if (o.obs && !(WG_ABLATE & 16)) {
        constexpr int d = IN3D ? 3 : 2, per = 3 * d;
        const int stride = o.obs_stride, nmid = kp.conmid ? 3 : 0;
        typedef float fvd __attribute__((ext_vector_type(d), aligned(4)));
        if (is_mass) {
            const float *rd = kp.midform == 2 ? s_red + 8 * mw : s_mid + 3 * mw;
            float *dst = WG_ST(o.obs, (uint32_t)s_row[mw] * (uint32_t)stride + per * (lane - mlm), 1);
            const float pm[3] = {px, py, pz}, vm[3] = {vx, vy, vz}, am[3] = {ax, ay, az};
            fvd vp, vv, va;
#pragma unroll
            for (int c = 0; c < d; c++) {
                const float mid = rd[c];
                vp[c] = kp.midform ? (pm[c] - mid) * kp.pk : pm[c] * kp.pk;
                vv[c] = vm[c] * kp.vk;
                va[c] = am[c] * kp.ak;
            }
            *reinterpret_cast<fvd *>(dst) = vp;
            *reinterpret_cast<fvd *>(dst + d) = vv;
            *reinterpret_cast<fvd *>(dst + 2 * d) = va;
        }
        if (lane < nw && nmid) {
            const int M = s_mo[lane + 1] - s_mo[lane];
            float *row = WG_ST(o.obs, (uint32_t)wrow * (uint32_t)stride + per * M, 1);
            const float *rd = s_red + 8 * lane;
            for (int c = 0; c < 3; c++) row[c] = kp.midform == 2 ? rd[c] : kp.midform ? rd[c] / (float)M : 0.f;
        }
        if (is_mus)
            *WG_ST(o.obs, (uint32_t)s_row[uw] * (uint32_t)stride + per * (s_mo[uw + 1] - s_mo[uw]) + nmid + ua, 1) =
                x * kp.mk;
        if (!o.obs_pad_clean) {
            const float inv = 1.f / (float)stride;
            for (int i = lane; i < nw * stride; i += 64) {
                const int w = fdiv(i, stride, inv), c = i - w * stride;
                const int len = per * (s_mo[w + 1] - s_mo[w]) + nmid + (s_uo[w + 1] - s_uo[w]);
                if (c >= len) *WG_ST(o.obs, (uint32_t)s_row[w] * (uint32_t)stride + c, 1) = 0.f;
            }
        }
    }
    STAMP(6);
#ifdef WG_STAMPS
    if (lane == 0 && stamp_wave < (1 << 16)) {
        const unsigned hw = __builtin_amdgcn_s_getreg((31 << 11) | 4);
        const unsigned xcc = __builtin_amdgcn_s_getreg((31 << 11) | 20);
        g_stamps[stamp_wave * 8 + 7] = (unsigned long long)hw | ((unsigned long long)xcc << 32);
    }
#endif
}

__global__ void walker_reset_kernel(wg_batch b, const float *__restrict__ noise, const uint8_t *__restrict__ mask,
                                    int zmode) {
    const int P = b.ragged ? b.mass_off[b.N] : b.N * b.M;
    for (int q = blockIdx.x * blockDim.x + threadIdx.x; q < P; q += gridDim.x * blockDim.x) {
        int w;
        if (b.ragged) {
            int lo = 0, hi = b.N - 1;
            while (lo < hi) { const int mid = (lo + hi + 1) >> 1; if (b.mass_off[mid] <= q) lo = mid; else hi = mid - 1; }
            w = lo;
        } else {
            w = q / b.M;
        }
        if (mask && !mask[w]) continue;
        if (noise) {
#pragma unroll
            for (int c = 0; c < 3; c++) {
                const float n = noise[3 * q + c];
                const bool add = zmode == 2 ? __float_as_uint(n) != 0u : (c < 2 || zmode == 1);
                if (add) b.vel[3 * q + c] = b.vel[3 * q + c] + n;
            }
        }
    }
    for (int w = blockIdx.x * blockDim.x + threadIdx.x; w < b.N; w += gridDim.x * blockDim.x)
        if (!mask || mask[w]) b.steps[w] = 0;
}

__global__ __launch_bounds__(256) void walker_info_kernel(wg_batch b, uint8_t *__restrict__ nonfinite,
                                                          float *__restrict__ momentum, const int32_t *__restrict__ plan,
                                                          int plan_blocks) {
    const int w = blockIdx.x * blockDim.x + threadIdx.x;
    if (w >= b.N) return;
    if (plan && (w < plan[0] || w >= plan[plan_blocks])) return;
    const int p0 = b.ragged ? b.mass_off[w] : w * b.M, p1 = b.ragged ? b.mass_off[w + 1] : p0 + b.M;
    float mx = 0.f, my = 0.f, mz = 0.f;
    bool bad = false;
    for (int q = p0; q < p1; q++) {
        const float *pv = b.pos + 3 * (size_t)q, *vv = b.vel + 3 * (size_t)q, *av = b.acc + 3 * (size_t)q;
        const float vx = vv[0], vy = vv[1], vz = vv[2], m = b.mass[q];
        bad = bad || !(__builtin_isfinite(pv[0]) && __builtin_isfinite(pv[1]) && __builtin_isfinite(pv[2]) &&
                       __builtin_isfinite(vx) && __builtin_isfinite(vy) && __builtin_isfinite(vz) &&
                       __builtin_isfinite(av[0]) && __builtin_isfinite(av[1]) && __builtin_isfinite(av[2]));
        mx = mx + vx * m; my = my + vy * m; mz = mz + vz * m;
    }
    const int r = caller_row(b, w);
    if (nonfinite) nonfinite[r] = (uint8_t)bad;
    if (momentum) { momentum[3 * r] = mx; momentum[3 * r + 1] = my; momentum[3 * r + 2] = mz; }
}

int env_int(const char *name, int dflt);
int wave_passes(int M, int K);

KParams make_kparams(const wg_params &p) {
    KParams k;
    k.neg_g = (float)(-p.g);
    k.neg_dampk = (float)(-p.dampk);
    k.ground = (float)p.ground;
    k.neg_groundk = (float)(-p.groundk);
    k.neg_grounddamp = (float)(-p.grounddamp);
    k.friction = (float)p.friction;
    k.dt = (float)p.dt;
    k.pk = (float)p.pk; k.vk = (float)p.vk; k.ak = (float)p.ak; k.mk = (float)p.mk;
    k.done_y = (float)(p.ground - 50.0);
    k.g = p.g;
    k.max_steps = p.max_steps; k.midform = p.midform; k.conmid = p.conmid;
    k.spring_mode = p.spring_mode; k.action_mode = p.action_mode;
    k.integrator = p.integrator;
    k.pair_mode = p.pair_mode;
    k.pair_g = p.pair_g;
    k.pair_k = p.pair_k;
    k.pair_e = p.pair_e;
    k.bounce_kh = (float)(p.bounce_k / 2);
    for (int i = 0; i < 3; i++) k.g3g[i] = (float)p.g3_gravity[i];
    k.g3_damp = (float)p.g3_damping;
    k.g3_dragc = (float)(-0.5 * p.g3_air);
    k.g3_level = (float)p.g3_ground_level;
    k.g3_rest = (float)p.g3_restitution;
    k.g3_fric = (float)p.g3_friction;
    k.g3_ground = p.g3_ground;
    k.friction_mode = p.friction_mode;
    k.prio = env_int("WG_LEAN_PRIO", 1);
    k.xcd = env_int("WG_XCD", 3);

    k.dt2 = (float)(p.dt * p.dt);
    return k;
}

constexpr int RAG_P = 256, RAG_E = 512, RAG_U = 256, RAG_W = 64;
constexpr int LDS_LIMIT = 160 * 1024;

int validate(const wg_batch *b) {
    if (!b) return fail(WG_EINVAL, "null batch");
    if (b->N < 0 || b->M < 1 || b->K < 0 || b->A < 0 || b->A > b->K)
        return fail(WG_EINVAL, "bad sizes N=%d M=%d K=%d A=%d", b->N, b->M, b->K, b->A);
    if (2 * b->K > 65535) return fail(WG_ERANGE, "K=%d exceeds the u16 incidence encoding", b->K);
    if (b->M > WG_MAX_M) return fail(WG_ERANGE, "M=%d > %d masses per walker", b->M, WG_MAX_M);
    if (!b->pos || !b->vel || !b->acc || !b->mass || !b->steps || !b->muscle_x)
        return fail(WG_EINVAL, "missing state pointer");
    if (b->K > 0 && (!b->edges || !b->inc || !b->inc_off)) return fail(WG_EINVAL, "missing edge pointer");
    if (b->M > 32767) return fail(WG_ERANGE, "M=%d exceeds the 15-bit edge endpoint encoding", b->M);
    if (!b->inc_off) return fail(WG_EINVAL, "missing inc_off");
    if (b->ragged < 0 || b->ragged > 2) return fail(WG_EINVAL, "ragged must be 0, 1 or 2");
    if (b->ragged && (!b->mass_off || !b->edge_off || !b->muscle_off))
        return fail(WG_EINVAL, "ragged batch without offsets");
    if (!b->ragged && b->row) return fail(WG_EINVAL, "row (a walker permutation) is for ragged batches only");
    if (b->ragged == 2 && !wave_passes(b->M, b->K))
        return fail(WG_EINVAL, "ragged = 2 (wave tiles) needs M <= 64 and at most 8 spring passes (M=%d K=%d)", b->M, b->K);
    return 0;
}

Geo uniform_geo(const wg_batch *b, int obs_stride, bool no_lite = false) {
    Geo g{};
    int W = std::max(1, NTHREADS / b->M);
    if (b->M > 64 && env_int("WG_WIDE", 1)) {
        int best = 0, bestT = NTHREADS;
        for (int T = NTHREADS; T <= MAXT; T += 64) {
            const int w = T / b->M;
            if (w >= 1 && (int64_t)w * b->M * bestT > (int64_t)best * T) { best = w * b->M; bestT = T; W = w; }
        }
    }
    if (b->K > 0) W = std::max(1, std::min(W, EPL * MAXT / std::max(1, b->K)));
    while (W > 1 && (b->N + W - 1) / W < 512) W = std::max(1, W / 2);
    g.W = W;
    const bool shfl_shape = b->M <= 64 && (64 % b->M) == 0 && !(WG_ABLATE & 64);
    for (;;) {
        g.Pcap = g.W * b->M; g.Ecap = g.W * b->K; g.Ucap = g.W * b->A;
        g.tbytes = std::max(g.Ecap * 3 * 8, g.W * std::max(0, obs_stride) * 4);
        g.lite = (shfl_shape && g.W * b->M <= MAXT && !no_lite) ? 1 : 0;
        g.threads = std::min(MAXT, std::max(64, ((g.W * b->M + 63) / 64) * 64));
        if (b->K > 0 && g.W * b->K > EPL * g.threads) g.threads = MAXT;
        g.lds = carve_bytes(g);
        if (g.lds <= 64 * 1024 || g.W == 1) break;
        g.W = std::max(1, g.W / 2);
    }
    g.invM = 1.f / (float)b->M;
    g.invK = 1.f / (float)std::max(1, b->K);
    g.invA = 1.f / (float)std::max(1, b->A);
    return g;
}

Geo ragged_geo(const wg_batch *b) {
    Geo g{};
    g.threads = NTHREADS;
    g.W = RAG_W;
    g.Pcap = std::max(RAG_P, b->M);
    g.Ecap = std::max(RAG_E, b->K);
    g.Ucap = std::max(RAG_U, b->A);
    g.tbytes = g.Ecap * 3 * 8;
    g.lite = 0;
    g.lds = carve_bytes(g);
    g.invM = g.invK = g.invA = 0.f;
    return g;
}

template <bool STEP, bool RAGGED, bool IN3D, int PWD, bool SHFL>
int launch(const wg_batch *b, const KParams &kp, const float *action, int cols, int astride,
           const wg_outputs &o, const int32_t *plan, int blocks, const Geo &g, hipStream_t stream) {
    const int lds_static = (int)(sizeof(s_pw_log2) + sizeof(s_pw_exp2));
    if (g.lds + lds_static > LDS_LIMIT)
        return fail(WG_ERANGE, "workgroup needs %d B of LDS (> 160 KiB)", g.lds + lds_static);
    WG_KLAUNCH((walker_step_kernel<STEP, RAGGED, IN3D, PWD, SHFL>), dim3(blocks), dim3(g.threads), (uint32_t)g.lds, stream,
               *b, kp, action, cols, astride, kout(o), plan, g);
    const hipError_t e = hipGetLastError();
    if (e != hipSuccess) return fail(WG_EHIP, "launch failed: %s", hipGetErrorString(e));
    return 0;
}

bool shfl_ok(const wg_batch *b, const Geo &g) { return !b->ragged && g.lite; }

template <bool STEP, int PWD>
int dispatch2(const wg_batch *b, const KParams &kp, bool in3d, const float *a, int cols, int astride,
              const wg_outputs &o, const int32_t *plan, int blocks, const Geo &g, hipStream_t st) {
    if (b->ragged) {
        return in3d ? launch<STEP, true, true, PWD, false>(b, kp, a, cols, astride, o, plan, blocks, g, st)
                    : launch<STEP, true, false, PWD, false>(b, kp, a, cols, astride, o, plan, blocks, g, st);
    }
    if (PWD == 0 && shfl_ok(b, g)) {
        return in3d ? launch<STEP, false, true, 0, true>(b, kp, a, cols, astride, o, plan, blocks, g, st)
                    : launch<STEP, false, false, 0, true>(b, kp, a, cols, astride, o, plan, blocks, g, st);
    }
    return in3d ? launch<STEP, false, true, PWD, false>(b, kp, a, cols, astride, o, plan, blocks, g, st)
                : launch<STEP, false, false, PWD, false>(b, kp, a, cols, astride, o, plan, blocks, g, st);
}
int env_int(const char *name, int dflt) {
    const char *e = getenv(name);
    return (e && *e) ? atoi(e) : dflt;
}

bool lean_enabled() { return env_int("WG_LEAN", 1) != 0; }

bool u32_bytes(const wg_batch *b) {
    const int64_t lim = 1ll << 32;
    return (int64_t)b->N * b->M * 12 < lim && (int64_t)b->N * b->K * 16 < lim && (int64_t)b->N * b->A * 8 < lim &&
           (int64_t)b->N * (b->M + 1) * 2 < lim;
}
bool obs_u32(const wg_batch *b, int obs_stride) { return (int64_t)b->N * std::max(obs_stride, 1) * 4 < (1ll << 32); }

bool lean_geo(const wg_batch *b, int obs_stride, LeanGeo *out, int spring_mode = 0) {
    const int M = b->M;
    if (b->ragged || M < 4 || M > 64 || (64 % M) != 0 || b->K < 1 || !lean_enabled() || (WG_ABLATE & 128)) return false;
    if (spring_mode != 0) return false;
    if ((int64_t)b->N * b->M * 3 >= (1ll << 31) || (int64_t)b->N * b->K * 4 >= (1ll << 31) ||
        !obs_u32(b, obs_stride) || !u32_bytes(b))
        return false;
    LeanGeo g{};
    g.wpw = 64 / M;
    while (g.wpw > 1 && (b->N + g.wpw - 1) / g.wpw < 512) g.wpw >>= 1;
    const int wcap = env_int("WG_LEAN_WPW", 0);
    if (wcap > 0 && wcap < g.wpw) g.wpw = wcap;
    g.lgM = 0;
    while ((1 << g.lgM) < M) g.lgM++;
    if ((g.wpw * b->K + 63) / 64 > 8 || g.wpw * b->A > 64) return false;
    const int wpb = env_int("WG_LEAN_WAVES", 0);
    g.wpb = (wpb == 1 || wpb == 2 || wpb == 4) ? wpb : ((b->N + g.wpw - 1) / g.wpw <= 1024 ? 1 : 4);
    const int ew = g.wpw * b->K;
    g.pl = (ew + 3) & ~3;
    g.off_df = align16(g.pl * 24);
    g.off_inc = g.off_df + align16(g.pl * 12);
    g.off_x = g.off_inc + align16(ew * 4 + 4);
    g.slice = g.off_x + align16(std::max(1, g.wpw * b->A) * 4);
    if (4 * g.slice > 80 * 1024) return false;
    g.invK = 1.f / (float)b->K;
    g.invA = 1.f / (float)std::max(1, b->A);
    g.invM = 1.f / (float)M;
    g.nblk = (b->N + g.wpb * g.wpw - 1) / (g.wpb * g.wpw);
    *out = g;
    return true;
}

int lean_blocks(const wg_batch *b, const LeanGeo &g) { return (b->N + g.wpb * g.wpw - 1) / (g.wpb * g.wpw); }

int launch_lean(const wg_batch *b, const KParams &kp, bool in3d, const float *a, int cols, int astride,
                const wg_outputs &o, const LeanGeo &g, hipStream_t st) {
    const int blocks = lean_blocks(b, g);
    const int ne = (g.wpw * b->K + 63) / 64;
    const int lds = g.wpb * g.slice + std::max(0, env_int("WG_LDS_PAD", 0));
#define WG_LAUNCH_LEAN(D3, NE_)                                                                                  \
    WG_KLAUNCH((walker_step_lean<D3, NE_>), dim3(blocks), dim3(64 * g.wpb), (uint32_t)lds, st, *b, kp, a, cols,  \
               astride, kout(o), g)
#define WG_LEAN_NE(D3)                                                         \
    do {                                                                       \
        if (ne == 2) WG_LAUNCH_LEAN(D3, 2);                                    \
        else if (ne == 3) WG_LAUNCH_LEAN(D3, 3);                               \
        else if (ne == 4) WG_LAUNCH_LEAN(D3, 4);                               \
        else WG_LAUNCH_LEAN(D3, 8);                                            \
    } while (0)
    if (ne <= 1) {
        if (in3d)
            WG_KLAUNCH((walker_step_lean1<true>), dim3(blocks), dim3(64 * g.wpb), (uint32_t)lds, st, b->pos, b->vel,
                               b->edges, b->inc, b->N, b->M, b->K, g.wpw, g.wpb, (int)((unsigned)g.nblk | ((unsigned)(kp.xcd & 2) << 29) | ((unsigned)(kp.prio != 0) << 31)), *b,
                               kp, a, cols, astride, kout(o), g);
        else
            WG_KLAUNCH((walker_step_lean1<false>), dim3(blocks), dim3(64 * g.wpb), (uint32_t)lds, st, b->pos, b->vel,
                               b->edges, b->inc, b->N, b->M, b->K, g.wpw, g.wpb, (int)((unsigned)g.nblk | ((unsigned)(kp.xcd & 2) << 29) | ((unsigned)(kp.prio != 0) << 31)), *b,
                               kp, a, cols, astride, kout(o), g);
    } else if (in3d) {
        WG_LEAN_NE(true);
    } else {
        WG_LEAN_NE(false);
    }
#undef WG_LEAN_NE
#undef WG_LAUNCH_LEAN
    const hipError_t e = hipGetLastError();
    if (e != hipSuccess) return fail(WG_EHIP, "launch failed: %s", hipGetErrorString(e));
    return 0;
}

int launch_lean_rollout(const wg_batch *b, const KParams &kp, bool in3d, const float *a, int cols, int astride,
                        int64_t astep, const wg_outputs &o, int n_steps, const LeanGeo &g, hipStream_t st) {
    const int blocks = lean_blocks(b, g);
    const int ne = (g.wpw * b->K + 63) / 64;
    const int lds = g.wpb * g.slice;
#define WG_LAUNCH_RO(D3, NE_)                                                                                    \
    hipLaunchKernelGGL((walker_rollout_lean<D3, NE_>), dim3(blocks), dim3(64 * g.wpb), lds, st, *b, kp, a, cols, \
                       astride, astep, kout(o), n_steps, g)
#define WG_RO_NE(D3)                                                                                             \
    do {                                                                                                         \
        if (ne <= 1) WG_LAUNCH_RO(D3, 1);                                                                        \
        else if (ne == 2) WG_LAUNCH_RO(D3, 2);                                                                   \
        else if (ne == 3) WG_LAUNCH_RO(D3, 3);                                                                   \
        else if (ne == 4) WG_LAUNCH_RO(D3, 4);                                                                   \
        else WG_LAUNCH_RO(D3, 8);                                                                                \
    } while (0)
    if (in3d) WG_RO_NE(true); else WG_RO_NE(false);
#undef WG_RO_NE
#undef WG_LAUNCH_RO
    const hipError_t e = hipGetLastError();
    if (e != hipSuccess) return fail(WG_EHIP, "launch failed: %s", hipGetErrorString(e));
    return 0;
}

int wave_passes(int M, int K) {
    if (M < 1 || M > 64 || K < 0) return 0;
    int ne = std::max((K + 63) / 64, (K + M - 1) / M);
    ne = std::max(ne, 1);
    if (ne > 8) return 0;
    return ne <= 4 ? ne : 8;
}

bool rag_geo(const wg_batch *b, int obs_stride, RagGeo *out) {
    const int ne = wave_passes(b->M, b->K);
    if (b->ragged != 2 || ne == 0 || b->A > 64 || !u32_bytes(b) || !obs_u32(b, obs_stride)) return false;
    RagGeo g{};
    const int wpb = env_int("WG_LEAN_WAVES", 4);
    g.wpb = (wpb == 1 || wpb == 2) ? wpb : 4;
    const int ec = 64 * ne;
    g.off_df = align16(std::max(ec * 24, 4 * 64 * 6));
    g.off_inc = g.off_df + align16(std::max(ec * 12, 4 * RW_MAXW * 8));
    g.off_x = g.off_inc + align16(ec * 4 + 4);
    g.off_wo = g.off_x + align16(64 * 4);
    g.slice = g.off_wo + align16(4 * (RW_MAXW + 1) * 3 + 4 * RW_MAXW + 12 * RW_MAXW);
    *out = g;
    return true;
}

int launch_waves(const wg_batch *b, const KParams &kp, bool in3d, const float *a, int cols, int astride,
                 const wg_outputs &o, const int32_t *plan, int ntiles, const RagGeo &g, hipStream_t st) {
    const int ne = wave_passes(b->M, b->K);
    const int blocks = (ntiles + g.wpb - 1) / g.wpb;
    const int lds = g.wpb * g.slice;
#define WG_LAUNCH_WAVES(D3, NE_)                                                                                  \
    WG_KLAUNCH((walker_step_waves<D3, NE_>), dim3(blocks), dim3(64 * g.wpb), (uint32_t)lds, st, *b, kp, a, cols,   \
               astride, kout(o), plan, ntiles, g)
#define WG_WAVES_NE(D3)                                                        \
    do {                                                                       \
        if (ne <= 1) WG_LAUNCH_WAVES(D3, 1);                                   \
        else if (ne == 2) WG_LAUNCH_WAVES(D3, 2);                              \
        else if (ne == 3) WG_LAUNCH_WAVES(D3, 3);                              \
        else if (ne == 4) WG_LAUNCH_WAVES(D3, 4);                              \
        else WG_LAUNCH_WAVES(D3, 8);                                           \
    } while (0)
    if (in3d) WG_WAVES_NE(true); else WG_WAVES_NE(false);
#undef WG_WAVES_NE
#undef WG_LAUNCH_WAVES
    const hipError_t e = hipGetLastError();
    if (e != hipSuccess) return fail(WG_EHIP, "launch failed: %s", hipGetErrorString(e));
    return 0;
}

int reset_impl(const wg_batch *b, const float *noise, const uint8_t *mask, int zmode, hipStream_t stream) {
    int rc = validate(b);
    if (rc) return rc;
    if (b->N == 0) return 0;
    const long P = b->ragged ? -1 : (long)b->N * b->M;
    const int blocks = P > 0 ? (int)std::min<long>((P + 255) / 256, 4096) : 1024;
    hipLaunchKernelGGL(walker_reset_kernel, dim3(blocks), dim3(256), 0, stream, *b, noise, mask, zmode);
    const hipError_t e = hipGetLastError();
    if (e != hipSuccess) return fail(WG_EHIP, "reset launch failed: %s", hipGetErrorString(e));
    return 0;
}

template <bool STEP>
int dispatch(const wg_batch *b, const KParams &kp, bool in3d, const float *a, int cols, int astride,
             const wg_outputs &o, const int32_t *plan, int blocks, const Geo &g, hipStream_t st) {
    return b->M <= 128 ? dispatch2<STEP, 0>(b, kp, in3d, a, cols, astride, o, plan, blocks, g, st)
                       : dispatch2<STEP, 3>(b, kp, in3d, a, cols, astride, o, plan, blocks, g, st);
}

int run(const wg_batch *b, const wg_params *p, const float *action, int32_t cols, int32_t astride,
        int64_t astep, const wg_outputs *o, int32_t n_steps, const int32_t *plan, int32_t plan_blocks,
        hipStream_t stream, bool step, bool resident = false, bool check_only = false, int s_first = 0) {
    int rc = validate(b);
    if (rc) return rc;
    if (!p) return fail(WG_EINVAL, "null params");
    if (b->N == 0 || n_steps <= 0) return 0;
    if (action && (cols < 0 || astride < cols)) return fail(WG_EINVAL, "bad action stride");
    if (action && p->action_mode == 1 && !b->muscle_stride) return fail(WG_EINVAL, "discrete actions need muscle_stride");
    if (p->integrator < 0 || p->integrator > 2) return fail(WG_EINVAL, "integrator must be 0/1 (run1) or 2 (run2)");
    if (action && !b->muscle_bounds) return fail(WG_EINVAL, "actions need muscle_bounds");
    if (b->ragged && (!plan || plan_blocks <= 0)) return fail(WG_EINVAL, "ragged batch needs a plan");
    wg_outputs out = o ? *o : wg_outputs{};
    if (out.obs && out.obs_stride <= 0) return fail(WG_EINVAL, "obs_stride must be > 0");
    const KParams kp = make_kparams(*p);
    const Geo g = b->ragged ? ragged_geo(b) : uniform_geo(b, out.obs ? out.obs_stride : 0, step && p->pair_mode != 0);
    if (g.W > g.threads) return fail(WG_ERANGE, "more than %d walkers per workgroup", g.threads);
    const int blocks = b->ragged ? plan_blocks : (b->N + g.W - 1) / g.W;
    LeanGeo lg{};
    const bool act_u32 = !action || (int64_t)b->N * astride * 4 < (1ll << 32);
    const bool use_lean = step && act_u32 && lean_geo(b, out.obs ? out.obs_stride : 0, &lg, p->spring_mode);
    RagGeo rgeo{};
    const bool use_waves = step && act_u32 && p->spring_mode == 0 && p->pair_mode == 0 && lean_enabled() &&
                           rag_geo(b, out.obs ? out.obs_stride : 0, &rgeo);
    if (p->spring_mode < 0 || p->spring_mode > 2)
        return fail(WG_EINVAL, "spring_mode %d: 0 (engine.py), 1 (G2 element), 2 (G3 engine) only", p->spring_mode);
    if (step && (p->pair_mode & ~31))
        return fail(WG_EINVAL, "pair_mode %d: bits 1 (gravity), 2 (coulomb), 4 (bounce), 8 (G2 gravity_vec), "
                               "16 (electrostatic) only", p->pair_mode);
    if (step && p->pair_mode != 0 && p->spring_mode != 0)
        return fail(WG_EINVAL, "pair_mode %d needs spring_mode 0", p->pair_mode);
    if (step && (p->pair_mode & 4) && !b->radius)
        return fail(WG_EINVAL, "pair_mode 4 (bounce) needs the radius array");
    if (check_only) return 0;
    const bool extras = out.nonfinite || out.momentum;
    auto info_pass = [&](const wg_outputs &os) -> int {
        if (!(os.nonfinite || os.momentum)) return 0;
        hipLaunchKernelGGL(walker_info_kernel, dim3((b->N + 255) / 256), dim3(256), 0, stream, *b, os.nonfinite,
                           os.momentum, b->ragged ? plan : nullptr, plan_blocks);
        const hipError_t e = hipGetLastError();
        return e == hipSuccess ? 0 : fail(WG_EHIP, "info launch failed: %s", hipGetErrorString(e));
    };
    if (resident && use_lean && p->pair_mode == 0 && !extras)
        return launch_lean_rollout(b, kp, p->in3d != 0, action, cols, astride, action ? astep : 0, out, n_steps, lg,
                                   stream);
    for (int s = s_first; s < s_first + n_steps; s++) {
        wg_outputs os = out;
        if (os.obs) os.obs += s * os.obs_step;
        if (os.reward) os.reward += s * os.out_step;
        if (os.done) os.done += s * os.out_step;
        if (os.energy) os.energy += s * os.out_step;
        if (os.centroid) os.centroid += 3 * s * os.out_step;
        if (os.steps) os.steps += s * os.out_step;
        if (os.nonfinite) os.nonfinite += s * os.out_step;
        if (os.momentum) os.momentum += 3 * s * os.out_step;
        const float *a = action ? action + s * astep : nullptr;
        if (step && use_lean) rc = launch_lean(b, kp, p->in3d != 0, a, cols, astride, os, lg, stream);
        else if (use_waves) rc = launch_waves(b, kp, p->in3d != 0, a, cols, astride, os, plan, plan_blocks, rgeo, stream);
        else rc = step ? dispatch<true>(b, kp, p->in3d != 0, a, cols, astride, os, plan, blocks, g, stream)
                       : dispatch<false>(b, kp, p->in3d != 0, nullptr, 0, 0, os, plan, blocks, g, stream);
        if (rc) return rc;
        if (extras && (rc = info_pass(os))) return rc;
    }
    return 0;
}

__global__ __launch_bounds__(1024) void floor_empty_kernel(float *) {}
__global__ __launch_bounds__(1024) void floor_load_store_kernel(const float *__restrict__ in, float *__restrict__ out) {
    const size_t i = (size_t)blockIdx.x * blockDim.x + threadIdx.x;
    out[i] = in[i] + 1.0f;
}
__global__ __launch_bounds__(1024) void floor_busy_kernel(const float *__restrict__ in, float *__restrict__ out) {
    const size_t i = (size_t)blockIdx.x * blockDim.x + threadIdx.x;
    float x = in[i], y = 0.5f;
#pragma unroll 16
    for (int k = 0; k < 4096; k++) y = __builtin_fmaf(y, 0.99993896484375f, x);
    out[i] = y;
}

}

extern "C" {

int wg_abi_version(void) { return WG_ABI_VERSION; }
const char *wg_last_error(void) { return g_err; }

int wg_step(const wg_batch *b, const wg_params *p, const float *action, int32_t action_cols,
            int32_t action_stride, int64_t action_step, const wg_outputs *o, int32_t n_steps,
            const int32_t *plan, int32_t plan_blocks, hipStream_t stream) {
    return run(b, p, action, action_cols, action_stride, action_step, o, n_steps, plan, plan_blocks, stream, true);
}

int wg_rollout(const wg_batch *b, const wg_params *p, const float *action, int32_t action_cols,
               int32_t action_stride, int64_t action_step, const wg_outputs *o, int32_t n_steps,
               const int32_t *plan, int32_t plan_blocks, hipStream_t stream) {
    return run(b, p, action, action_cols, action_stride, action_step, o, n_steps, plan, plan_blocks, stream, true,
               true);
}

int wg_run_ranges(const wg_range *ranges, int32_t n, const wg_params *p, const float *action, int32_t action_cols,
                  int32_t action_stride, int64_t action_step, int32_t n_steps, hipEvent_t *events) {
    if (!ranges || n < 1 || (n > 1 && !events)) return fail(WG_EINVAL, "wg_run_ranges: bad ranges / events");
    for (int i = 0; i < n; i++) {
        const wg_range &r = ranges[i];
        const int rc = run(r.batch, p, action ? action + r.action_offset : nullptr, action_cols, action_stride,
                           action_step, r.outputs, n_steps, r.plan, r.plan_blocks, r.stream, true, false, true);
        if (rc) return rc;
    }
    if (n_steps <= 0) return 0;
    hipStream_t s0 = ranges[0].stream;
    if (n > 1 && hipEventRecord(events[0], s0) != hipSuccess) return fail(WG_EHIP, "fork event record failed");
    for (int i = 1; i < n; i++)
        if (hipStreamWaitEvent(ranges[i].stream, events[0], 0) != hipSuccess) return fail(WG_EHIP, "fork wait failed");
    auto issue = [&](int i, int s) -> int {
        const wg_range &r = ranges[i];
        return run(r.batch, p, action ? action + r.action_offset : nullptr, action_cols, action_stride, action_step,
                   r.outputs, 1, r.plan, r.plan_blocks, r.stream, true, false, false, s);
    };
    int rc = 0;
    for (int s = 0; s < n_steps && !rc; s++)
        for (int i = 0; i < n && !rc; i++) rc = issue(i, s);
    for (int i = 1; i < n; i++)
        if (hipEventRecord(events[i], ranges[i].stream) != hipSuccess || hipStreamWaitEvent(s0, events[i], 0) != hipSuccess)
            return rc ? rc : fail(WG_EHIP, "join event failed");
    return rc;
}

int wg_step_ranges(const wg_range *ranges, int32_t n, const wg_params *p, const float *action, int32_t action_cols,
                   int32_t action_stride, hipEvent_t *events) {
    return wg_run_ranges(ranges, n, p, action, action_cols, action_stride, 0, 1, events);
}

int wg_observe(const wg_batch *b, const wg_params *p, const wg_outputs *o, const int32_t *plan,
               int32_t plan_blocks, hipStream_t stream) {
    if (!o) return fail(WG_EINVAL, "null outputs");
    return run(b, p, nullptr, 0, 0, 0, o, 1, plan, plan_blocks, stream, false);
}

int wg_step_simple(const wg_batch *b, const float *action, const wg_params *p, int32_t n_steps, hipStream_t stream) {
    if (b && b->ragged) return fail(WG_EINVAL, "wg_step_simple: uniform batches only (ragged: wg_step with a plan)");
    const int32_t A = b ? b->A : 0;
    const int64_t step = b ? (int64_t)b->N * A : 0;
    return run(b, p, A > 0 ? action : nullptr, A, A, step, nullptr, n_steps, nullptr, 0, stream, true);
}

int wg_observe_simple(const wg_batch *b, const wg_obs_cfg *cfg, float *obs, float *reward, uint8_t *done,
                      float *centroid, float *energy, hipStream_t stream) {
    if (b && b->ragged) return fail(WG_EINVAL, "wg_observe_simple: uniform batches only (ragged: wg_observe with a plan)");
    if (!b || !cfg) return fail(WG_EINVAL, "null batch / cfg");
    wg_outputs o{};
    o.obs = obs;
    o.obs_stride = 3 * (cfg->in3d ? 3 : 2) * b->M + (cfg->conmid ? 3 : 0) + b->A;
    o.reward = reward;
    o.done = done;
    o.centroid = centroid;
    o.energy = energy;
    return run(b, cfg, nullptr, 0, 0, 0, &o, 1, nullptr, 0, stream, false);
}

int wg_time_step(const wg_batch *b, const wg_params *p, const float *action, int32_t action_cols, int32_t action_stride,
                 int64_t action_step, const wg_outputs *o, int32_t n_steps, const int32_t *plan, int32_t plan_blocks,
                 hipStream_t stream, float *ms_per_launch) {
    if (!ms_per_launch || n_steps < 1) return fail(WG_EINVAL, "wg_time_step: n_steps >= 1 and ms_per_launch required");
    int rc = run(b, p, action, action_cols, action_stride, action_step, o, n_steps, plan, plan_blocks, stream, true,
                 false, true);
    if (rc) return rc;
    if (b->N == 0) return fail(WG_EINVAL, "wg_time_step: empty batch (no launch to time)");
    std::vector<hipEvent_t> ev((size_t)2 * n_steps, nullptr);
    for (auto &e : ev)
        if (hipEventCreate(&e) != hipSuccess) { rc = fail(WG_EHIP, "wg_time_step: event create failed"); break; }
    for (int s = 0; s < n_steps && !rc; s++) {
        g_kev_start = ev[2 * s]; g_kev_stop = ev[2 * s + 1];
        rc = run(b, p, action, action_cols, action_stride, action_step, o, 1, plan, plan_blocks, stream, true, false,
                 false, s);
    }
    g_kev_start = g_kev_stop = nullptr;
    double total = 0.0;
    if (hipStreamSynchronize(stream) != hipSuccess && !rc) rc = fail(WG_EHIP, "wg_time_step: stream sync failed");
    for (int s = 0; s < n_steps && !rc; s++) {
        float ms = 0.f;
        if (hipEventElapsedTime(&ms, ev[2 * s], ev[2 * s + 1]) != hipSuccess)
            rc = fail(WG_EHIP, "wg_time_step: elapsed time of step %d unavailable", s);
        total += ms;
    }
    for (auto e : ev)
        if (e) (void)hipEventDestroy(e);
    if (!rc) *ms_per_launch = (float)(total / n_steps);
    return rc;
}

int wg_reset(const wg_batch *b, const wg_params *p, const float *noise, const uint8_t *mask, hipStream_t stream) {
    if (!p) return fail(WG_EINVAL, "null params");
    return reset_impl(b, noise, mask, p->in3d ? 1 : 0, stream);
}

int wg_reset_noise(const wg_batch *b, const float *noise, hipStream_t stream) {
    return reset_impl(b, noise, nullptr, 2, stream);
}

int wg_wave_edge_passes(int32_t M, int32_t K) { return wave_passes(M, K); }

int wg_plan_errors(int32_t clear) {
    int v = 0;
    if (hipMemcpyFromSymbol(&v, HIP_SYMBOL(g_plan_error), sizeof v, 0, hipMemcpyDeviceToHost) != hipSuccess)
        return fail(WG_EHIP, "plan error flag copy failed");
    if (clear && v) {
        const int z = 0;
        if (hipMemcpyToSymbol(HIP_SYMBOL(g_plan_error), &z, sizeof z, 0, hipMemcpyHostToDevice) != hipSuccess)
            return fail(WG_EHIP, "plan error flag reset failed");
    }
    return v;
}

int wg_plan_waves(const int32_t *mass_off, const int32_t *edge_off, const int32_t *muscle_off, int32_t N,
                  int32_t *plan, int32_t max_tiles) {
    if (!mass_off || !edge_off || !muscle_off || !plan || N < 0 || max_tiles < 1)
        return fail(WG_EINVAL, "bad plan args");
    int Mmax = 1, Kmax = 0;
    for (int w = 0; w < N; w++) {
        Mmax = std::max(Mmax, mass_off[w + 1] - mass_off[w]);
        Kmax = std::max(Kmax, edge_off[w + 1] - edge_off[w]);
    }
    const int ne = wave_passes(Mmax, Kmax);
    if (!ne) return fail(WG_EINVAL, "a walker does not fit one wave (M=%d K=%d)", Mmax, Kmax);
    int tiles = 0, w = 0;
    plan[0] = 0;
    while (w < N) {
        int P = 0, E = 0, U = 0, n = 0;
        while (w < N) {
            const int m = mass_off[w + 1] - mass_off[w], k = edge_off[w + 1] - edge_off[w],
                      a = muscle_off[w + 1] - muscle_off[w];
            if (m > 64 || a > 64 || k > 64 * ne) return fail(WG_EINVAL, "walker %d does not fit one wave", w);
            if (n > 0 && (P + m > 64 || E + k > 64 * ne || U + a > 64 || n + 1 > RW_MAXW)) break;
            P += m; E += k; U += a; n++; w++;
        }
        if (tiles + 1 > max_tiles) return fail(WG_ERANGE, "plan needs more than %d tiles", max_tiles);
        plan[++tiles] = w;
    }
    return tiles;
}

int wg_plan_ragged(const int32_t *mass_off, const int32_t *edge_off, const int32_t *muscle_off,
                   int32_t N, int32_t *plan, int32_t max_blocks) {
    if (!mass_off || !edge_off || !muscle_off || !plan || N < 0 || max_blocks < 1)
        return fail(WG_EINVAL, "bad plan args");
    int blocks = 0;
    plan[0] = 0;
    int w = 0;
    while (w < N) {
        int P = 0, E = 0, U = 0, n = 0;
        while (w < N) {
            const int m = mass_off[w + 1] - mass_off[w], k = edge_off[w + 1] - edge_off[w],
                      a = muscle_off[w + 1] - muscle_off[w];
            if (n > 0 && (P + m > RAG_P || E + k > RAG_E || U + a > RAG_U || n + 1 > RAG_W)) break;
            P += m; E += k; U += a; n++; w++;
        }
        if (blocks + 1 > max_blocks) return fail(WG_ERANGE, "plan needs more than %d blocks", max_blocks);
        plan[++blocks] = w;
    }
    return blocks;
}

int wg_launch_floor(int32_t mode, int32_t blocks, int32_t threads, const float *in, float *out, int32_t n_launches,
                    hipStream_t stream) {
    if (blocks < 1 || threads < 1 || threads > 1024 || n_launches < 0 || mode < 0 || mode > 2 ||
        (mode >= 1 && (!in || !out)))
        return fail(WG_EINVAL, "bad floor launch (mode %d, %d x %d)", mode, blocks, threads);
    for (int i = 0; i < n_launches; i++) {
        if (mode == 0)
            hipLaunchKernelGGL(floor_empty_kernel, dim3(blocks), dim3(threads), 0, stream, out);
        else if (mode == 1)
            hipLaunchKernelGGL(floor_load_store_kernel, dim3(blocks), dim3(threads), 0, stream, in, out);
        else
            hipLaunchKernelGGL(floor_busy_kernel, dim3(blocks), dim3(threads), 0, stream, in, out);
    }
    return hipGetLastError() == hipSuccess ? 0 : fail(WG_EHIP, "floor launch failed");
}

int wg_debug_stamps(unsigned long long *host, int n) {
#ifdef WG_STAMPS
    if (hipMemcpyFromSymbol(host, HIP_SYMBOL(g_stamps), (size_t)n * 8 * sizeof(unsigned long long), 0,
                            hipMemcpyDeviceToHost) != hipSuccess)
        return fail(WG_EHIP, "stamp copy failed");
    return 0;
#else
    (void)host; (void)n;
    return fail(WG_EINVAL, "not a stamps build");
#endif
}

int wg_launch_geometry(const wg_batch *b, wg_launch_info *info) {
    int rc = validate(b);
    if (rc) return rc;
    if (!info) return fail(WG_EINVAL, "null info");
    LeanGeo lg{};
    if (lean_geo(b, 0, &lg)) {
        info->threads = 64 * lg.wpb;
        info->walkers_per_block = lg.wpb * lg.wpw;
        info->blocks = lean_blocks(b, lg);
        info->lds_bytes = lg.wpb * lg.slice;
        return 0;
    }
    RagGeo rg{};
    if (b->ragged == 2 && lean_enabled() && rag_geo(b, 0, &rg)) {
        info->threads = 64 * rg.wpb;
        info->walkers_per_block = -1;
        info->blocks = -1;
        info->lds_bytes = rg.wpb * rg.slice;
        return 0;
    }
    const Geo g = b->ragged ? ragged_geo(b) : uniform_geo(b, 0);
    info->threads = g.threads;
    info->walkers_per_block = g.W;
    info->blocks = b->ragged ? -1 : (b->N + g.W - 1) / g.W;
    info->lds_bytes = g.lds;
    return 0;
}

}
```

walker_gym_amd/device.py:

```python
from __future__ import annotations

import ctypes as C
import os
from typing import Optional

import numpy as np
import torch

from . import _lib
from .layout import HostLayout, default_radius


def _to_dev(a: np.ndarray, device) -> torch.Tensor:
    a = np.ascontiguousarray(a)
    if a.dtype == np.uint16:
        t = torch.from_numpy(a.view(np.int16))
    elif a.dtype == np.uint32:
        t = torch.from_numpy(a.view(np.int32))
    else:
        t = torch.from_numpy(a)
    return t.to(device, non_blocking=False).contiguous()


def _ptr(t: Optional[torch.Tensor]):
    return None if t is None else C.c_void_p(t.data_ptr())


class DeviceBatch:

    STATE = ("pos", "vel", "acc", "muscle_x", "steps")

    def __init__(self, host: HostLayout, device: torch.device, contact: bool = True, wave_ok: bool = True):
        if device.type != "cuda":
            raise ValueError("DeviceBatch needs a ROCm device (torch 'cuda' device); there is no CPU path")
        self.host = host
        self.device = device
        self.N, self.M, self.K, self.A, self.ragged = host.N, host.M, host.K, host.A, host.ragged
        self.P, self.E, self.U = host.P, host.E, host.U
        dv = device
        self.mass_off = _to_dev(host.mass_off, dv)
        self.edge_off = _to_dev(host.edge_off, dv)
        self.muscle_off = _to_dev(host.muscle_off, dv)
        self.pos = _to_dev(host.pos, dv)
        self.vel = _to_dev(host.vel, dv)
        self.acc = _to_dev(host.acc, dv)
        self.mass = _to_dev(host.mass, dv)
        self.edges = _to_dev(host.edges, dv)
        self.inc = _to_dev(host.inc, dv) if host.E else None
        self.inc_off = _to_dev(host.inc_off, dv)
        self.muscle_x = _to_dev(host.muscle_x, dv)
        self.muscle_bounds = _to_dev(host.muscle_bounds, dv)
        self.muscle_stride = _to_dev(host.muscle_stride, dv)
        self.steps = _to_dev(host.steps, dv)
        self.contact = torch.zeros(self.P, dtype=torch.uint8, device=dv) if contact else None
        self.pinned = _to_dev(host.pinned, dv) if host.pinned is not None else None
        self.charge = _to_dev(host.charge, dv) if host.charge is not None else None
        self.bounce_set = _to_dev(host.bounce_set, dv) if host.bounce_set is not None else None
        self.radius = None
        self._dummy = torch.zeros(16, dtype=torch.float32, device=dv)
        self.row = _to_dev(host.row, dv) if host.row is not None else None
        self._perm = {}
        if host.row is not None:
            inv = np.empty(self.N, np.int64)
            inv[host.row] = np.arange(self.N)
            self._perm = {"walker": torch.from_numpy(inv).to(dv), "row": torch.from_numpy(host.row.astype(np.int64)).to(dv),
                          "mass": torch.from_numpy(host.mass_perm).to(dv),
                          "muscle": torch.from_numpy(host.muscle_perm).to(dv)}
        self.plan = None
        self.plan_blocks = 0
        self.ragged_kind = 0
        self.version = 0
        self.replan(wave_ok)

    def replan(self, wave_ok: bool) -> None:
        host, L = self.host, _lib.load()
        self.wave_ok = bool(wave_ok)
        lean_shape = 4 <= self.M <= 64 and 64 % self.M == 0
        self.ragged = host.ragged
        self.plan, self.plan_host, self.plan_blocks, self.ragged_kind = None, None, 0, 0
        waves = (wave_ok and self.A <= 64 and L.wg_wave_edge_passes(self.M, self.K) > 0
                 and os.environ.get("WG_LEAN", "1") != "0")
        if (not self.ragged and not lean_shape and waves and os.environ.get("WG_UNIFORM_WAVES", "1") != "0"):
            self.ragged = True
        if self.ragged:
            plan = np.zeros(self.N + 1, np.int32)
            args = (host.mass_off.ctypes.data_as(C.c_void_p), host.edge_off.ctypes.data_as(C.c_void_p),
                    host.muscle_off.ctypes.data_as(C.c_void_p), self.N, plan.ctypes.data_as(C.c_void_p), self.N + 1)
            if waves:
                nb, self.ragged_kind = _lib.check(L.wg_plan_waves(*args), "wg_plan_waves"), 2
            else:
                nb, self.ragged_kind = _lib.check(L.wg_plan_ragged(*args), "wg_plan_ragged"), 1
            self.plan = _to_dev(plan[:nb + 1], self.device)
            self.plan_host = plan[:nb + 1].copy()
            self.plan_blocks = nb
        self.struct = self._make_struct()

    def caller(self, name: str) -> torch.Tensor:
        t = getattr(self, name)
        if t is None or not self._perm:
            return t
        return t.index_select(0, self._perm[self.KIND[name]])

    def stored_mass(self, q: int) -> int:
        return int(self.host.mass_perm[q]) if self._perm else int(q)

    def to_stored(self, kind: str, t: torch.Tensor) -> torch.Tensor:
        if not self._perm:
            return t
        if kind == "walker":
            return t.index_select(0, self._perm["row"])
        if kind not in ("mass", "muscle"):
            raise ValueError(f"to_stored: kind must be 'mass', 'muscle' or 'walker', not {kind!r}")
        out = torch.empty_like(t)
        out.index_copy_(0, self._perm[kind], t)
        return out

    def enable_radius(self) -> None:
        if self.radius is None:
            r = self.host.radius if self.host.radius is not None else default_radius(self.host.mass)
            self.radius = _to_dev(r, self.device)
            self.struct = self._make_struct()

    def _p(self, t):
        if t is None:
            return None
        if t.numel() == 0:
            return C.c_void_p(self._dummy.data_ptr())
        return C.c_void_p(t.data_ptr())

    def _make_struct(self) -> _lib.WgBatch:
        r = self.ragged
        return _lib.WgBatch(
            N=self.N, M=self.M, K=self.K, A=self.A, ragged=self.ragged_kind if r else 0, row=self._p(self.row),
            mass_off=self._p(self.mass_off) if r else None, edge_off=self._p(self.edge_off) if r else None,
            muscle_off=self._p(self.muscle_off) if r else None,
            pos=self._p(self.pos), vel=self._p(self.vel), acc=self._p(self.acc), mass=self._p(self.mass),
            edges=self._p(self.edges),
            inc=self._p(self.inc) if self.inc is not None else None, inc_off=self._p(self.inc_off),
            muscle_x=self._p(self.muscle_x), muscle_bounds=self._p(self.muscle_bounds),
            muscle_stride=self._p(self.muscle_stride), steps=self._p(self.steps), contact=self._p(self.contact),
            pinned=self._p(self.pinned), charge=self._p(self.charge), radius=self._p(self.radius),
            bounce_set=self._p(self.bounce_set))

    def sub_struct(self, w0: int, w1: int) -> _lib.WgBatch:
        if self.ragged:
            raise ValueError("sub_struct: uniform batches only")
        if not 0 <= w0 < w1 <= self.N:
            raise ValueError(f"sub_struct: bad walker range [{w0}, {w1})")
        M, K, A = self.M, self.K, self.A

        def off(t, elems):
            return None if t is None else C.c_void_p(t.data_ptr() + elems * t.element_size())

        return _lib.WgBatch(
            N=w1 - w0, M=M, K=K, A=A, ragged=0, mass_off=None, edge_off=None, muscle_off=None,
            pos=off(self.pos, 3 * M * w0), vel=off(self.vel, 3 * M * w0), acc=off(self.acc, 3 * M * w0),
            mass=off(self.mass, M * w0), edges=off(self.edges, 4 * K * w0),
            inc=off(self.inc, 2 * K * w0) if self.inc is not None else None,
            inc_off=off(self.inc_off, (M + 1) * w0),
            muscle_x=self._p(self.muscle_x) if A == 0 else off(self.muscle_x, A * w0),
            muscle_bounds=self._p(self.muscle_bounds) if A == 0 else off(self.muscle_bounds, 2 * A * w0),
            muscle_stride=self._p(self.muscle_stride) if A == 0 else off(self.muscle_stride, A * w0),
            steps=off(self.steps, w0), contact=off(self.contact, M * w0), pinned=off(self.pinned, M * w0),
            charge=off(self.charge, M * w0), radius=off(self.radius, M * w0), row=None,
            bounce_set=off(self.bounce_set, M * w0))

    def launch_geometry(self) -> dict:
        info = _lib.WgLaunchInfo()
        _lib.check(_lib.load().wg_launch_geometry(C.byref(self.struct), C.byref(info)), "wg_launch_geometry")
        blocks = info.blocks
        if self.ragged:
            wpb = max(1, info.threads // 64)
            blocks = -(-self.plan_blocks // wpb) if self.ragged_kind == 2 else self.plan_blocks
        geo = dict(threads=info.threads, walkers_per_block=info.walkers_per_block, blocks=blocks,
                   lds_bytes=info.lds_bytes)
        if self.ragged_kind == 2:
            geo["wave_tiles"] = self.plan_blocks
        return geo

    KIND = {"pos": "mass", "vel": "mass", "acc": "mass", "contact": "mass", "radius": "mass", "muscle_x": "muscle",
            "steps": "walker"}

    def state_dict(self) -> dict:
        sd = {k: self.caller(k).clone() for k in self.STATE}
        if self.radius is not None:
            sd["radius"] = self.caller("radius").clone()
        return sd

    def load_state_dict(self, sd: dict) -> None:
        self.version += 1
        for k in self.STATE:
            getattr(self, k).copy_(self.to_stored(self.KIND[k], sd[k].to(self.device)))
        if "radius" in sd:
            self.enable_radius()
            self.radius.copy_(self.to_stored("mass", sd["radius"].to(self.device)))
```

walker_gym_amd/layout.py:

```python
from __future__ import annotations

from dataclasses import dataclass, field
from typing import Dict, Optional

import os

import numpy as np

f32 = np.float32
SPEC_KEYS = ("m", "pos", "vel", "mass_off", "ei", "ej", "rest", "k", "c", "flags", "edge_off", "n_muscles",
             "minl", "maxl", "stride")


@dataclass
class HostLayout:
    N: int
    M: int
    K: int
    A: int
    ragged: bool
    mass_off: np.ndarray
    edge_off: np.ndarray
    muscle_off: np.ndarray
    pos: np.ndarray
    vel: np.ndarray
    acc: np.ndarray
    mass: np.ndarray
    edges: np.ndarray
    inc: np.ndarray
    inc_off: np.ndarray
    muscle_x: np.ndarray
    muscle_bounds: np.ndarray
    muscle_stride: np.ndarray
    steps: np.ndarray
    pinned: Optional[np.ndarray] = None
    charge: Optional[np.ndarray] = None
    radius: Optional[np.ndarray] = None
    bounce_set: Optional[np.ndarray] = None
    row: Optional[np.ndarray] = None
    mass_perm: Optional[np.ndarray] = None
    muscle_perm: Optional[np.ndarray] = None
    extra: Dict[str, np.ndarray] = field(default_factory=dict)

    @property
    def P(self) -> int:
        return int(self.mass_off[-1])

    @property
    def E(self) -> int:
        return int(self.edge_off[-1])

    @property
    def U(self) -> int:
        return int(self.muscle_off[-1])

    def obs_len(self, in3d: bool, conmid: bool) -> np.ndarray:
        d = 3 if in3d else 2
        n = (3 * d * np.diff(self.mass_off) + (3 if conmid else 0) + np.diff(self.muscle_off)).astype(np.int32)
        if self.row is None:
            return n
        out = np.empty_like(n)
        out[self.row] = n
        return out


def incidence(ei: np.ndarray, ej: np.ndarray, mass_off: np.ndarray, edge_off: np.ndarray):
    N = len(mass_off) - 1
    Ks = np.diff(edge_off).astype(np.int64)
    Ms = np.diff(mass_off).astype(np.int64)
    E = int(edge_off[-1])
    if E and (Ks.max() * 2 > 65535):
        raise ValueError("a walker with more than 32767 edges does not fit the u16 incidence encoding")
    wid = np.repeat(np.arange(N, dtype=np.int64), Ks)
    local_e = np.arange(E, dtype=np.int64) - np.repeat(edge_off[:-1].astype(np.int64), Ks)
    mass = np.stack([ei.astype(np.int64), ej.astype(np.int64)], 1).reshape(-1)
    end = np.tile(np.array([0, 1], np.int64), E)
    e2 = np.repeat(local_e, 2)
    w2 = np.repeat(wid, 2)
    if E and (mass.min() < 0 or np.any(mass >= np.repeat(Ms, 2 * Ks))):
        raise ValueError("edge endpoint out of range of its walker")
    maxk = int(Ks.max()) if N else 0
    key = ((w2 * (int(Ms.max()) + 1 if N else 1) + mass) * (2 * maxk + 2) + 2 * e2 + end)
    order = np.argsort(key, kind="stable")
    inc = ((e2[order] << 1) | end[order]).astype(np.uint16)
    counts = np.zeros(int(mass_off[-1]), np.int64)
    np.add.at(counts, np.repeat(mass_off[:-1].astype(np.int64), 2 * Ks) + mass, 1)
    inc_off = np.zeros(int(mass_off[-1]) + N, np.uint16)
    for_w = np.repeat(np.arange(N, dtype=np.int64), Ms)
    csum = np.cumsum(counts)
    start_w = np.concatenate([[0], csum])[mass_off[:-1].astype(np.int64)]
    excl = np.concatenate([[0], csum[:-1]]) - start_w[for_w]
    q_local = np.arange(int(mass_off[-1]), dtype=np.int64) - mass_off[:-1].astype(np.int64)[for_w]
    pos_in = mass_off[:-1].astype(np.int64)[for_w] + for_w + q_local
    inc_off[pos_in] = excl.astype(np.uint16)
    inc_off[(mass_off[1:].astype(np.int64) + np.arange(N))] = (2 * Ks).astype(np.uint16)
    return inc, inc_off


def pack(spec: Dict[str, np.ndarray], mx: Optional[np.ndarray] = None, steps: Optional[np.ndarray] = None,
         sort: bool = True) -> HostLayout:
    if mx is not None:
        spec = dict(spec, mx=mx)
    if steps is not None:
        spec = dict(spec, steps=steps)
    Ms, Ks = np.diff(np.asarray(spec["mass_off"])), np.diff(np.asarray(spec["edge_off"]))
    nm = np.asarray(spec["n_muscles"])
    uniform = len(Ms) > 0 and np.all(Ms == Ms[0]) and np.all(Ks == Ks[0]) and np.all(nm == nm[0])
    row = mass_perm = muscle_perm = None
    if sort and not uniform and len(Ms) > 1:
        order = size_order(spec)
        if np.any(order != np.arange(len(order))):
            spec = reorder_walkers(spec, order)
            if spec.get("steps") is not None:
                spec["steps"] = np.asarray(spec["steps"])[order]
            row, mass_perm, muscle_perm = order.astype(np.int32), spec["_mass_perm"], spec["_muscle_perm"]
    lay = _pack(spec, spec.get("mx"), spec.get("steps"))
    lay.row, lay.mass_perm, lay.muscle_perm = row, mass_perm, muscle_perm
    return lay


def _pack(spec: Dict[str, np.ndarray], mx: Optional[np.ndarray], steps: Optional[np.ndarray]) -> HostLayout:
    s = {k: np.asarray(spec[k]) for k in SPEC_KEYS}
    mass_off = np.ascontiguousarray(s["mass_off"], np.int32)
    edge_off = np.ascontiguousarray(s["edge_off"], np.int32)
    n_mus = np.ascontiguousarray(s["n_muscles"], np.int32)
    N = len(mass_off) - 1
    muscle_off = np.concatenate([[0], np.cumsum(n_mus)]).astype(np.int32)
    Ms, Ks = np.diff(mass_off), np.diff(edge_off)
    if N == 0:
        raise ValueError("empty batch")
    if np.any(Ms < 1):
        raise ValueError("every walker needs at least one mass")
    if np.any(n_mus > Ks):
        raise ValueError("a walker has more muscles than edges (muscles are the first edges)")
    if Ms.max() > 1024:
        raise ValueError("walkers with more than 1024 masses are not supported (WG_MAX_M)")
    ragged = not (np.all(Ms == Ms[0]) and np.all(Ks == Ks[0]) and np.all(n_mus == n_mus[0]))
    ei = np.ascontiguousarray(s["ei"], np.int64)
    ej = np.ascontiguousarray(s["ej"], np.int64)
    if Ms.max() > 32767:
        raise ValueError("walker-local mass index does not fit the 15-bit edge endpoint encoding")
    flags = np.ascontiguousarray(s["flags"], np.uint8)
    edge_ij = (ei.astype(np.uint32) | (ej.astype(np.uint32) << np.uint32(16))
               | ((flags & 1).astype(np.uint32) << np.uint32(31))).astype(np.uint32)
    inc, inc_off = incidence(ei, ej, mass_off, edge_off)
    rest = np.ascontiguousarray(s["rest"], f32)
    uw = np.repeat(np.arange(N), n_mus)
    medge = edge_off[:-1][uw] + (np.arange(int(muscle_off[-1])) - muscle_off[:-1][uw])
    x0 = rest[medge]
    minl = np.ascontiguousarray(s["minl"], f32)
    maxl = np.ascontiguousarray(s["maxl"], f32)
    lo = (x0 * minl).astype(f32)
    hi = (x0 * maxl).astype(f32)
    pos = np.ascontiguousarray(s["pos"], f32).reshape(-1, 3)
    acc = spec.get("acc")
    edges = np.stack([edge_ij, rest.view(np.uint32), np.ascontiguousarray(s["k"], f32).view(np.uint32),
                      np.ascontiguousarray(s["c"], f32).view(np.uint32)], axis=1) if len(rest) else \
        np.zeros((0, 4), np.uint32)
    return HostLayout(
        N=N, M=int(Ms.max()), K=int(Ks.max()), A=int(n_mus.max()), ragged=bool(ragged),
        mass_off=mass_off, edge_off=edge_off, muscle_off=muscle_off,
        pos=pos.copy(), vel=np.ascontiguousarray(s["vel"], f32).reshape(-1, 3).copy(),
        acc=(np.zeros_like(pos) if acc is None else np.ascontiguousarray(acc, f32).reshape(-1, 3).copy()),
        mass=np.ascontiguousarray(s["m"], f32), edges=np.ascontiguousarray(edges, np.uint32),
        inc=inc, inc_off=inc_off,
        muscle_x=(x0.copy() if mx is None else np.ascontiguousarray(mx, f32).copy()),
        muscle_bounds=np.ascontiguousarray(np.stack([lo, hi], axis=1).reshape(-1, 2), f32),
        muscle_stride=np.ascontiguousarray(s["stride"], f32),
        steps=(np.zeros(N, np.int32) if steps is None else np.ascontiguousarray(steps, np.int32).copy()),
        pinned=_pinned(spec, int(mass_off[-1])),
        charge=_per_mass_f64(spec, "charge", int(mass_off[-1])),
        radius=_per_mass_f64(spec, "radius", int(mass_off[-1])),
        bounce_set=_bounce_set(spec, int(mass_off[-1])),
    )


def _per_mass_f64(spec, key: str, P: int):
    a = spec.get(key)
    if a is None:
        return None
    a = np.ascontiguousarray(a, np.float64).reshape(-1)
    if a.shape[0] != P:
        raise ValueError(f"{key} has {a.shape[0]} entries for {P} masses")
    return a.copy()


def default_radius(mass: np.ndarray) -> np.ndarray:
    return np.asarray(mass, np.float32).astype(np.float64) ** 0.3


def bounce_set_from_lists(n_points: int, callers, other="*") -> np.ndarray:
    def idx(lst, what):
        a = np.asarray(list(lst), np.int64).reshape(-1)
        if a.size and (a.min() < 0 or a.max() >= n_points):
            raise ValueError(f"bounce {what}: point index out of range [0, {n_points})")
        if a.size > 1 and not bool(np.all(np.diff(a) > 0)):
            raise ValueError(f"bounce {what} must be in registry order (ascending point indices, no repeats): the "
                             "reference iterates the list as given, which bounce_set cannot express otherwise")
        return a
    bs = np.zeros(n_points, np.uint8)
    bs[idx(callers, "callers")] |= 1
    if isinstance(other, str):
        if other != "*":
            raise ValueError('bounce other must be "*" or a list of point indices')
        bs |= 2
    else:
        bs[idx(other, "other")] |= 2
    return bs


def _bounce_set(spec, P: int):
    bs = spec.get("bounce_set")
    if bs is None:
        return None
    bs = np.ascontiguousarray(bs).reshape(-1)
    if bs.shape[0] != P:
        raise ValueError(f"bounce_set has {bs.shape[0]} entries for {P} masses")
    if bs.size and (bs.min() < 0 or bs.max() > 3):
        raise ValueError("bounce_set entries are bit 0 (calls bounce) | bit 1 (in the other list): 0..3")
    bs = bs.astype(np.uint8)
    return None if bool(np.all(bs == 3)) else bs.copy()


def _pinned(spec, P: int):
    pin = spec.get("pinned")
    if pin is None:
        return None
    pin = np.ascontiguousarray(pin, np.uint8).reshape(-1)
    if pin.shape[0] != P:
        raise ValueError(f"pinned has {pin.shape[0]} entries for {P} masses")
    return (pin != 0).astype(np.uint8) if pin.any() else None


def reorder_walkers(spec: Dict[str, np.ndarray], order: np.ndarray) -> Dict[str, np.ndarray]:
    order = np.asarray(order, np.int64)
    mo, eo = np.asarray(spec["mass_off"], np.int64), np.asarray(spec["edge_off"], np.int64)
    nm = np.asarray(spec["n_muscles"], np.int64)
    uo = np.concatenate([[0], np.cumsum(nm)])

    def gather(off):
        lens = np.diff(off)[order]
        starts = off[:-1][order]
        idx = np.repeat(starts - np.concatenate([[0], np.cumsum(lens)[:-1]]), lens) + np.arange(int(lens.sum()))
        return idx, np.concatenate([[0], np.cumsum(lens)]).astype(np.int32)

    pidx, new_mo = gather(mo)
    eidx, new_eo = gather(eo)
    uidx, _ = gather(uo)
    out = dict(spec)
    for k in ("m", "pos", "vel", "acc", "pinned", "charge", "radius", "bounce_set"):
        if spec.get(k) is not None:
            out[k] = np.asarray(spec[k])[pidx]
    for k in ("ei", "ej", "rest", "k", "c", "flags"):
        out[k] = np.asarray(spec[k])[eidx]
    for k in ("minl", "maxl", "stride", "mx"):
        if spec.get(k) is not None:
            out[k] = np.asarray(spec[k])[uidx]
    out["mass_off"], out["edge_off"] = new_mo, new_eo
    out["n_muscles"] = nm[order].astype(np.int32)
    out["_mass_perm"] = np.empty(len(pidx), np.int64)
    out["_mass_perm"][pidx] = np.arange(len(pidx))
    out["_muscle_perm"] = np.empty(len(uidx), np.int64)
    out["_muscle_perm"][uidx] = np.arange(len(uidx))
    return out


WAVE_LANES = 64
WAVE_MAX_WALKERS = 32


def wave_edge_passes(M: int, K: int) -> int:
    if M < 1 or M > 64 or K < 0:
        return 0
    ne = max((K + 63) // 64, (K + M - 1) // M, 1)
    return 0 if ne > 8 else (ne if ne <= 4 else 8)


def wave_tile_order(M: np.ndarray, K: np.ndarray, A: np.ndarray, ne: int, window: Optional[int] = None) -> np.ndarray:
    if window is None:
        window = int(os.environ.get("WG_TILE_WINDOW", "512"))
    n = len(M)
    if window <= 0 or window >= n:
        return wave_tile_order_bfd(M, K, A, ne)
    parts = []
    for s in range(0, n, window):
        idx = np.arange(s, min(s + window, n))
        parts.append(idx[wave_tile_order_bfd(M[idx], K[idx], A[idx], ne)])
    return np.concatenate(parts)


def wave_tile_order_bfd(M: np.ndarray, K: np.ndarray, A: np.ndarray, ne: int) -> np.ndarray:
    n = len(M)
    order = np.lexsort((np.arange(n), -A, -K, -M))
    cap_e = WAVE_LANES * ne
    tiles = []
    free = [[] for _ in range(WAVE_LANES + 1)]
    for w in order.tolist():
        m, k, a = int(M[w]), int(K[w]), int(A[w])
        placed = False
        for r in range(m, WAVE_LANES + 1):
            lst = free[r]
            for j in range(len(lst) - 1, -1, -1):
                t = tiles[lst[j]]
                if t[1] + k <= cap_e and t[2] + a <= WAVE_LANES and t[3] < WAVE_MAX_WALKERS:
                    ti = lst.pop(j)
                    t[0] += m; t[1] += k; t[2] += a; t[3] += 1; t[4].append(w)
                    free[WAVE_LANES - t[0]].append(ti)
                    placed = True
                    break
            if placed:
                break
        if not placed:
            tiles.append([m, k, a, 1, [w]])
            free[WAVE_LANES - m].append(len(tiles) - 1)
    return np.fromiter((w for t in tiles for w in t[4]), np.int64, n)


def size_order(spec: Dict[str, np.ndarray]) -> np.ndarray:
    M = np.diff(np.asarray(spec["mass_off"], np.int64))
    K = np.diff(np.asarray(spec["edge_off"], np.int64))
    A = np.asarray(spec["n_muscles"], np.int64)
    if len(M):
        ne = wave_edge_passes(int(max(1, M.max())), int(K.max()))
        if ne and int(A.max()) <= WAVE_LANES and os.environ.get("WG_TILE_ORDER", "bfd") != "sorted":
            return wave_tile_order(M, K, A, ne)
    return np.lexsort((np.arange(len(M)), A, K, M))


def algorithmic_bytes_per_walker_step(M: int, K: int, A: int, obs_floats: int) -> int:
    return 64 * M + 16 * K + 20 * A + 8 + 4 * obs_floats


def layout_bytes_per_walker_step(M, K, A, obs_floats, info: bool = True, contact: bool = True,
                                 ragged: bool = False):
    b = algorithmic_bytes_per_walker_step(M, K, A, obs_floats)
    b = b + 2 * 2 * K + 2 * (M + 1) - 4 * A
    if info:
        b = b + 16
    if contact:
        b = b + M
    if ragged:
        b = b + 16
    return b
```

Before: 2.005 billion.

## Add compact 8-byte edge records and skip acc/contact stores on intermediate steps

Adds an 8-byte edge format that packs precomputed LDS byte offsets for both endpoints and the muscle slot, plus muscle and string flags, alongside the rest length. Per-class spring stiffness and damping move into a small constant array in the batch struct. This halves edge-load bandwidth and removes the per-edge division and index arithmetic in the lean kernels. Acceleration and contact writes are also skipped on non-final steps of multi-step runs, which cuts store traffic but means those buffers are only refreshed when needed. It applies only to uniform layouts where walkers exactly fill a wavefront and stiffness/damping are constant per class.

```diff
diff --git a/include/walker_hip.h b/include/walker_hip.h
--- a/include/walker_hip.h
+++ b/include/walker_hip.h
@@ -9,7 +9,7 @@
 typedef struct ihipStream_t *hipStream_t;
 typedef struct ihipEvent_t *hipEvent_t;
 
-#define WG_ABI_VERSION 14
+#define WG_ABI_VERSION 15
 #define WG_EINVAL (-1)
 #define WG_ERANGE (-2)
 #define WG_EHIP (-3)
@@ -43,6 +43,11 @@
     float rest, k, c;
 } wg_edge;
 
+typedef struct wg_edge8 {
+    uint32_t w;
+    float rest;
+} wg_edge8;
+
 typedef struct wg_batch {
     int32_t N, M, K, A;
     int32_t ragged;
@@ -62,6 +67,8 @@
     double *radius;
     const int32_t *row;
     const uint8_t *bounce_set;
+    const wg_edge8 *edges8;
+    float kc[4];
 } wg_batch;
 
 typedef struct wg_outputs {
diff --git a/walker_gym_amd/_lib.py b/walker_gym_amd/_lib.py
--- a/walker_gym_amd/_lib.py
+++ b/walker_gym_amd/_lib.py
@@ -7,7 +7,7 @@
 HERE = os.path.dirname(os.path.abspath(__file__))
 LIB_NAME = "libwalker_hip.so"
 LIB_PATH = os.path.join(HERE, LIB_NAME)
-ABI_VERSION = 14
+ABI_VERSION = 15
 
 WG_EINVAL, WG_ERANGE, WG_EHIP = -1, -2, -3
 
@@ -34,7 +34,8 @@
                 ("inc", _vp), ("inc_off", _vp),
                 ("muscle_x", _vp), ("muscle_bounds", _vp), ("muscle_stride", _vp),
                 ("steps", _vp), ("contact", _vp), ("pinned", _vp),
-                ("charge", _vp), ("radius", _vp), ("row", _vp), ("bounce_set", _vp)]
+                ("charge", _vp), ("radius", _vp), ("row", _vp), ("bounce_set", _vp),
+                ("edges8", _vp), ("kc", C.c_float * 4)]
 
 
 class WgOutputs(C.Structure):
diff --git a/walker_gym_amd/csrc/walker_hip.hip b/walker_gym_amd/csrc/walker_hip.hip
--- a/walker_gym_amd/csrc/walker_hip.hip
+++ b/walker_gym_amd/csrc/walker_hip.hip
@@ -8,6 +8,7 @@
 #include <cstdio>
 #include <cstdlib>
 #include <cstring>
+#include <type_traits>
 #include <vector>
 
 #include "walker_hip.h"
@@ -50,6 +51,7 @@
     int friction_mode;
     int prio;
     int xcd;
+    int keep_aux;
 };
 
 struct KOut {
@@ -1551,10 +1553,11 @@
     gt = gt || fexp3(g0, g1, g2) < TINY_EXP;
 }
 
-template <int NE>
+struct EdgeRec8 { uint32_t w; float rest; };
+template <int NE, bool E8 = false>
 struct LeanIn {
     float p3[3], v3[3];
-    EdgeRec er[NE];
+    typename std::conditional<E8, EdgeRec8, EdgeRec>::type er[NE];
     uint32_t gi[NE];
     float mf;
     int io0, io1, wsteps, pin;
@@ -1593,8 +1596,8 @@
 }
 #define WG_ST(base, e, n) (&at_u32w((base), (uint32_t)(n) * 4u * (uint32_t)(e)))
 __device__ __forceinline__ float neg_half_count(int n) { return -0.5f * (float)n; }
-template <int NE>
-__device__ __forceinline__ void lean_load_mass(const wg_batch &b, const LeanTile &t, int lane, LeanIn<NE> &L) {
+template <class LI>
+__device__ __forceinline__ void lean_load_mass(const wg_batch &b, const LeanTile &t, int lane, LI &L) {
     L.mf = 0.f; L.io0 = 0; L.io1 = 0; L.wsteps = 0; L.pin = 0;
     const int ln = min(lane, t.nP - 1);
     const int wl = ln >> (31 - __builtin_clz(b.M)), q = ln & (b.M - 1);
@@ -1604,9 +1607,9 @@
     L.io0 = at_u32(b.inc_off, 2u * io); L.io1 = at_u32(b.inc_off, 2u * io + 2u);
     L.wsteps = at_u32(b.steps, 4u * (uint32_t)(t.w0 + wl));
 }
-template <int NE>
+template <class LI>
 __device__ __forceinline__ void lean_load_muscles(const wg_batch &b, const KParams &kp, const float *__restrict__ action,
-                                                  int action_stride, const LeanTile &t, int lane, LeanIn<NE> &L) {
+                                                  int action_stride, const LeanTile &t, int lane, LI &L) {
     L.x = 0.f; L.lo = 0.f; L.hi = 0.f; L.stp = 0.f; L.a = 0.f;
     if (t.nU > 0) {
         const uint32_t ul = t.U0 + min(lane, t.nU - 1);
@@ -1620,9 +1623,9 @@
         }
     }
 }
-template <int NE>
+template <int NE, bool E8>
 __device__ __forceinline__ void lean_load(const wg_batch &b, const KParams &kp, const float *__restrict__ action,
-                                          int action_stride, const LeanTile &t, int lane, LeanIn<NE> &L) {
+                                          int action_stride, const LeanTile &t, int lane, LeanIn<NE, E8> &L) {
     const uint32_t pl = t.P0 + min(lane, t.nP - 1);
     const float *gp = &at_u32(b.pos, 12u * pl), *gv = &at_u32(b.vel, 12u * pl);
     L.p3[0] = gp[0]; L.p3[1] = gp[1]; L.p3[2] = gp[2];
@@ -1630,12 +1633,17 @@
 #pragma unroll
     for (int it = 0; it < NE; it++) {
         const uint32_t le = t.E0 + (uint32_t)min(lane + 64 * it, t.nE - 1);
-        const uint4 v = at_u32(reinterpret_cast<const uint4 *>(b.edges), 16u * le);
-        L.er[it] = EdgeRec{v.x, __uint_as_float(v.y), __uint_as_float(v.z), __uint_as_float(v.w)};
+        if constexpr (E8) {
+            const uint2 v = at_u32(reinterpret_cast<const uint2 *>(b.edges8), 8u * le);
+            L.er[it] = EdgeRec8{v.x, __uint_as_float(v.y)};
+        } else {
+            const uint4 v = at_u32(reinterpret_cast<const uint4 *>(b.edges), 16u * le);
+            L.er[it] = EdgeRec{v.x, __uint_as_float(v.y), __uint_as_float(v.z), __uint_as_float(v.w)};
+        }
         L.gi[it] = at_u32(reinterpret_cast<const uint32_t *>(b.inc), 4u * le);
     }
-    lean_load_mass<NE>(b, t, lane, L);
-    lean_load_muscles<NE>(b, kp, action, action_stride, t, lane, L);
+    lean_load_mass(b, t, lane, L);
+    lean_load_muscles(b, kp, action, action_stride, t, lane, L);
     if (!t.is_mass) {
         L.p3[0] = 0.f; L.p3[1] = 0.f; L.p3[2] = 0.f; L.v3[0] = 0.f; L.v3[1] = 0.f; L.v3[2] = 0.f;
         L.mf = 0.f; L.pin = 0; L.io0 = 0; L.io1 = 0;
@@ -1799,10 +1807,10 @@
     return TermsAoS{reinterpret_cast<double *>(sl), reinterpret_cast<float *>(sl + lg.off_df)};
 }
 
-template <bool IN3D, int NE, bool RES = false>
+template <bool IN3D, int NE, bool RES = false, bool E8 = false>
 __device__ __forceinline__ void lean_compute(const wg_batch &b, const KParams &kp, const KOut &o,
                                              const LeanGeo &lg, char *sl, const LeanTile &t, int lane,
-                                             LeanIn<NE> &L, bool last = true) {
+                                             LeanIn<NE, E8> &L, bool last = true) {
     const bool store = !RES || last;
     const int M = b.M, K = b.K, A = b.A;
     const int w0 = t.w0, nE = t.nE;
@@ -1860,10 +1868,16 @@
     const bool pos_ok = __all(fexp3(L.p3[0], L.p3[1], L.p3[2]) >= -55);
     struct Gath { float v[12]; };
     auto gather = [&](int it, Gath &g) {
-        const int le = lane + 64 * it;
-        const int ewl = fdiv(le, K, lg.invK);
-        const uint32_t ij = L.er[it].ij;
-        const int bi = ((ewl << lg.lgM) + edge_i(ij)) << 2, bj = ((ewl << lg.lgM) + edge_j(ij)) << 2;
+        int bi, bj;
+        if constexpr (E8) {
+            const uint32_t w = L.er[it].w;
+            bi = (int)w; bj = (int)(w >> 8);
+        } else {
+            const int le = lane + 64 * it;
+            const int ewl = fdiv(le, K, lg.invK);
+            const uint32_t ij = L.er[it].ij;
+            bi = ((ewl << lg.lgM) + edge_i(ij)) << 2; bj = ((ewl << lg.lgM) + edge_j(ij)) << 2;
+        }
 #pragma unroll
         for (int c = 0; c < 3; c++) {
             if (WG_ABLATE & 512) {
@@ -1876,11 +1890,21 @@
     };
     auto spring = [&](int it, const Gath &g) {
         const int le = lane + 64 * it;
-        const EdgeRec e = L.er[it];
-        const int ewl = fdiv(le, K, lg.invK), ew = le - (int)__umul24(ewl, K);
-        const bool mus = le < nE && ew < A;
-        const float xs = s_x[mus ? (int)__umul24(ewl, A) + ew : 0];
-        const float xr = mus ? xs : e.rest;
+        EdgeRec e;
+        float xr;
+        if constexpr (E8) {
+            const uint32_t w = L.er[it].w;
+            const bool mus = (w & 0x40000000u) != 0u;
+            const float xs = *reinterpret_cast<const float *>(reinterpret_cast<const char *>(s_x) + ((w >> 16) & 0xfcu));
+            xr = mus ? xs : L.er[it].rest;
+            e = EdgeRec{w, L.er[it].rest, mus ? b.kc[0] : b.kc[2], mus ? b.kc[1] : b.kc[3]};
+        } else {
+            e = L.er[it];
+            const int ewl = fdiv(le, K, lg.invK), ew = le - (int)__umul24(ewl, K);
+            const bool mus = le < nE && ew < A;
+            const float xs = s_x[mus ? (int)__umul24(ewl, A) + ew : 0];
+            xr = mus ? xs : e.rest;
+        }
         if (le < nE) {
             if (WG_ABLATE & 1) {
                 ts.put(le, xr + g.v[0] + g.v[3] + g.v[6] + g.v[9], g.v[1] + g.v[4] + g.v[7] + g.v[10],
@@ -1954,8 +1978,10 @@
             float *gpo = WG_ST(b.pos, pl, 3), *gvo = WG_ST(b.vel, pl, 3), *gao = WG_ST(b.acc, pl, 3);
             gpo[0] = px; gpo[1] = py; gpo[2] = pz;
             gvo[0] = vx; gvo[1] = vy; gvo[2] = vz;
-            gao[0] = ax; gao[1] = ay; gao[2] = az;
-            if (b.contact) at_u32w(b.contact, pl) = (uint8_t)hit;
+            if (RES || kp.keep_aux) {
+                gao[0] = ax; gao[1] = ay; gao[2] = az;
+                if (b.contact) at_u32w(b.contact, pl) = (uint8_t)hit;
+            }
         }
         if (q == 0) {
             const uint32_t wg = (uint32_t)(w0 + wl);
@@ -2030,7 +2056,7 @@
 
 constexpr int lean_waves(int NE) { return NE >= 8 ? 4 : 6; }
 
-template <bool IN3D, int NE>
+template <bool IN3D, int NE, bool E8>
 __global__ __launch_bounds__(256) __attribute__((amdgpu_waves_per_eu(lean_waves(NE)))) void walker_step_lean(
     wg_batch b, KParams kp, const float *__restrict__ action, int action_cols, int action_stride, KOut o,
     LeanGeo lg) {
@@ -2044,20 +2070,22 @@
 #endif
     STAMP(0);
     const LeanTile t = lean_tile_of(b, action, action_cols, lg, tile, lane);
-    LeanIn<NE> L;
+    LeanIn<NE, E8> L;
     if (kp.prio) __builtin_amdgcn_s_setprio(2);
-    lean_load<NE>(b, kp, action, action_stride, t, lane, L);
+    lean_load<NE, E8>(b, kp, action, action_stride, t, lane, L);
     if (kp.prio) __builtin_amdgcn_s_setprio(0);
     STAMP(1);
-    lean_compute<IN3D, NE>(b, kp, o, lg, smem + wv * lg.slice, t, lane, L);
-}
-
-template <bool IN3D>
+    lean_compute<IN3D, NE, false, E8>(b, kp, o, lg, smem + wv * lg.slice, t, lane, L);
+}
+
+template <bool IN3D, bool E8>
 __global__ __launch_bounds__(256) __attribute__((amdgpu_waves_per_eu(lean_waves(1)))) void walker_step_lean1(
-    float *pos, float *vel, const wg_edge *edges, const uint16_t *inc, int N, int M, int K, int wpw, int wpb, int nblkx,
+    float *pos, float *vel, const void *edges, const uint16_t *inc, int N, int M, int K, int wpw, int wpb, int nblkx,
     wg_batch b, KParams kp, const float *__restrict__ action, int action_cols, int action_stride, KOut o, LeanGeo lg) {
     extern __shared__ __attribute__((aligned(16))) char smem[];
-    b.pos = pos; b.vel = vel; b.edges = edges; b.inc = inc; b.N = N; b.M = M; b.K = K;
+    b.pos = pos; b.vel = vel; b.inc = inc; b.N = N; b.M = M; b.K = K;
+    if (E8) b.edges8 = static_cast<const wg_edge8 *>(edges);
+    else b.edges = static_cast<const wg_edge *>(edges);
     lg.nblk = nblkx & 0x3fffffff; lg.wpw = wpw; lg.wpb = wpb;
     kp.prio = (int)((unsigned)nblkx >> 31);
     const int lane = threadIdx.x & 63, wv = __builtin_amdgcn_readfirstlane(threadIdx.x >> 6);
@@ -2070,15 +2098,15 @@
 #endif
     STAMP(0);
     const LeanTile t = lean_tile_of(b, action, action_cols, lg, tile, lane);
-    LeanIn<1> L;
+    LeanIn<1, E8> L;
     if (kp.prio) __builtin_amdgcn_s_setprio(2);
-    lean_load<1>(b, kp, action, action_stride, t, lane, L);
+    lean_load<1, E8>(b, kp, action, action_stride, t, lane, L);
     if (kp.prio) __builtin_amdgcn_s_setprio(0);
     STAMP(1);
-    lean_compute<IN3D, 1>(b, kp, o, lg, smem + wv * lg.slice, t, lane, L);
-}
-
-template <bool IN3D, int NE>
+    lean_compute<IN3D, 1, false, E8>(b, kp, o, lg, smem + wv * lg.slice, t, lane, L);
+}
+
+template <bool IN3D, int NE, bool E8>
 __global__ __launch_bounds__(256) __attribute__((amdgpu_waves_per_eu(NE >= 8 ? 4 : 5))) void walker_rollout_lean(
     wg_batch b, KParams kp, const float *__restrict__ action, int action_cols, int action_stride, int64_t action_step,
     KOut o, int n_steps, LeanGeo lg) {
@@ -2090,9 +2118,9 @@
     const int stamp_wave = tile;
 #endif
     const LeanTile t = lean_tile_of(b, action, action_cols, lg, tile, lane);
-    LeanIn<NE> L;
+    LeanIn<NE, E8> L;
     if (kp.prio) __builtin_amdgcn_s_setprio(2);
-    lean_load<NE>(b, kp, action, action_stride, t, lane, L);
+    lean_load<NE, E8>(b, kp, action, action_stride, t, lane, L);
     if (kp.prio) __builtin_amdgcn_s_setprio(0);
     {
         uint32_t *s_inc = reinterpret_cast<uint32_t *>(smem + wv * lg.slice + lg.off_inc);
@@ -2118,9 +2146,11 @@
         if (os.steps) os.steps += (size_t)s * os.out_step;
         asm volatile("" : "+v"(L.mf), "+v"(L.io0), "+v"(L.io1), "+v"(L.lo), "+v"(L.hi), "+v"(L.stp));
 #pragma unroll
-        for (int it = 0; it < NE; it++) asm volatile("" : "+v"(L.er[it].ij), "+v"(L.er[it].rest), "+v"(L.er[it].k),
-                                                     "+v"(L.er[it].c));
-        lean_compute<IN3D, NE, true>(b, kp, os, lg, smem + wv * lg.slice, ts, ln, L, s == n_steps - 1);
+        for (int it = 0; it < NE; it++) {
+            if constexpr (E8) asm volatile("" : "+v"(L.er[it].w), "+v"(L.er[it].rest));
+            else asm volatile("" : "+v"(L.er[it].ij), "+v"(L.er[it].rest), "+v"(L.er[it].k), "+v"(L.er[it].c));
+        }
+        lean_compute<IN3D, NE, true, E8>(b, kp, os, lg, smem + wv * lg.slice, ts, ln, L, s == n_steps - 1);
         L.a = a_next;
         wave_sync();
     }
@@ -2314,8 +2344,10 @@
         float *gpo = WG_ST(b.pos, pl, 3), *gvo = WG_ST(b.vel, pl, 3), *gao = WG_ST(b.acc, pl, 3);
         gpo[0] = px; gpo[1] = py; gpo[2] = pz;
         gvo[0] = vx; gvo[1] = vy; gvo[2] = vz;
-        gao[0] = ax; gao[1] = ay; gao[2] = az;
-        if (b.contact) at_u32w(b.contact, pl) = (uint8_t)hit;
+        if (kp.keep_aux) {
+            gao[0] = ax; gao[1] = ay; gao[2] = az;
+            if (b.contact) at_u32w(b.contact, pl) = (uint8_t)hit;
+        }
         if (b.radius) b.radius[pl] = hit ? 3.0 : 1.0;
     }
     STAMP(4);
@@ -2506,6 +2538,7 @@
     k.friction_mode = p.friction_mode;
     k.prio = env_int("WG_LEAN_PRIO", 1);
     k.xcd = env_int("WG_XCD", 3);
+    k.keep_aux = 1;
 
     k.dt2 = (float)(p.dt * p.dt);
     return k;
@@ -2613,6 +2646,10 @@
 }
 
 bool lean_enabled() { return env_int("WG_LEAN", 1) != 0; }
+
+bool use_edge8(const wg_batch *b, const LeanGeo &g) {
+    return b->edges8 != nullptr && g.wpw * b->M == 64 && env_int("WG_EDGE8", 1) != 0;
+}
 
 bool u32_bytes(const wg_batch *b) {
     const int64_t lim = 1ll << 32;
@@ -2660,30 +2697,32 @@
     const int blocks = lean_blocks(b, g);
     const int ne = (g.wpw * b->K + 63) / 64;
     const int lds = g.wpb * g.slice + std::max(0, env_int("WG_LDS_PAD", 0));
-#define WG_LAUNCH_LEAN(D3, NE_)                                                                                  \
-    WG_KLAUNCH((walker_step_lean<D3, NE_>), dim3(blocks), dim3(64 * g.wpb), (uint32_t)lds, st, *b, kp, a, cols,  \
-               astride, kout(o), g)
-#define WG_LEAN_NE(D3)                                                         \
+    const bool e8 = use_edge8(b, g);
+#define WG_LAUNCH_LEAN(D3, NE_, E8_)                                                                             \
+    WG_KLAUNCH((walker_step_lean<D3, NE_, E8_>), dim3(blocks), dim3(64 * g.wpb), (uint32_t)lds, st, *b, kp, a,   \
+               cols, astride, kout(o), g)
+#define WG_LEAN_NE(D3, E8_)                                                    \
     do {                                                                       \
-        if (ne == 2) WG_LAUNCH_LEAN(D3, 2);                                    \
-        else if (ne == 3) WG_LAUNCH_LEAN(D3, 3);                               \
-        else if (ne == 4) WG_LAUNCH_LEAN(D3, 4);                               \
-        else WG_LAUNCH_LEAN(D3, 8);                                            \
+        if (ne == 2) WG_LAUNCH_LEAN(D3, 2, E8_);                               \
+        else if (ne == 3) WG_LAUNCH_LEAN(D3, 3, E8_);                          \
+        else if (ne == 4) WG_LAUNCH_LEAN(D3, 4, E8_);                          \
+        else WG_LAUNCH_LEAN(D3, 8, E8_);                                       \
     } while (0)
+#define WG_LAUNCH_LEAN1(D3, E8_)                                                                                 \
+    WG_KLAUNCH((walker_step_lean1<D3, E8_>), dim3(blocks), dim3(64 * g.wpb), (uint32_t)lds, st, b->pos, b->vel,  \
+               (E8_) ? static_cast<const void *>(b->edges8) : static_cast<const void *>(b->edges), b->inc, b->N, \
+               b->M, b->K, g.wpw, g.wpb,                                                                         \
+               (int)((unsigned)g.nblk | ((unsigned)(kp.xcd & 2) << 29) | ((unsigned)(kp.prio != 0) << 31)), *b,  \
+               kp, a, cols, astride, kout(o), g)
     if (ne <= 1) {
-        if (in3d)
-            WG_KLAUNCH((walker_step_lean1<true>), dim3(blocks), dim3(64 * g.wpb), (uint32_t)lds, st, b->pos, b->vel,
-                               b->edges, b->inc, b->N, b->M, b->K, g.wpw, g.wpb, (int)((unsigned)g.nblk | ((unsigned)(kp.xcd & 2) << 29) | ((unsigned)(kp.prio != 0) << 31)), *b,
-                               kp, a, cols, astride, kout(o), g);
-        else
-            WG_KLAUNCH((walker_step_lean1<false>), dim3(blocks), dim3(64 * g.wpb), (uint32_t)lds, st, b->pos, b->vel,
-                               b->edges, b->inc, b->N, b->M, b->K, g.wpw, g.wpb, (int)((unsigned)g.nblk | ((unsigned)(kp.xcd & 2) << 29) | ((unsigned)(kp.prio != 0) << 31)), *b,
-                               kp, a, cols, astride, kout(o), g);
+        if (in3d) { if (e8) WG_LAUNCH_LEAN1(true, true); else WG_LAUNCH_LEAN1(true, false); }
+        else { if (e8) WG_LAUNCH_LEAN1(false, true); else WG_LAUNCH_LEAN1(false, false); }
     } else if (in3d) {
-        WG_LEAN_NE(true);
+        if (e8) WG_LEAN_NE(true, true); else WG_LEAN_NE(true, false);
     } else {
-        WG_LEAN_NE(false);
-    }
+        if (e8) WG_LEAN_NE(false, true); else WG_LEAN_NE(false, false);
+    }
+#undef WG_LAUNCH_LEAN1
 #undef WG_LEAN_NE
 #undef WG_LAUNCH_LEAN
     const hipError_t e = hipGetLastError();
@@ -2696,18 +2735,20 @@
     const int blocks = lean_blocks(b, g);
     const int ne = (g.wpw * b->K + 63) / 64;
     const int lds = g.wpb * g.slice;
-#define WG_LAUNCH_RO(D3, NE_)                                                                                    \
-    hipLaunchKernelGGL((walker_rollout_lean<D3, NE_>), dim3(blocks), dim3(64 * g.wpb), lds, st, *b, kp, a, cols, \
-                       astride, astep, kout(o), n_steps, g)
-#define WG_RO_NE(D3)                                                                                             \
+    const bool e8 = use_edge8(b, g);
+#define WG_LAUNCH_RO(D3, NE_, E8_)                                                                               \
+    hipLaunchKernelGGL((walker_rollout_lean<D3, NE_, E8_>), dim3(blocks), dim3(64 * g.wpb), lds, st, *b, kp, a,  \
+                       cols, astride, astep, kout(o), n_steps, g)
+#define WG_RO_NE(D3, E8_)                                                                                        \
     do {                                                                                                         \
-        if (ne <= 1) WG_LAUNCH_RO(D3, 1);                                                                        \
-        else if (ne == 2) WG_LAUNCH_RO(D3, 2);                                                                   \
-        else if (ne == 3) WG_LAUNCH_RO(D3, 3);                                                                   \
-        else if (ne == 4) WG_LAUNCH_RO(D3, 4);                                                                   \
-        else WG_LAUNCH_RO(D3, 8);                                                                                \
+        if (ne <= 1) WG_LAUNCH_RO(D3, 1, E8_);                                                                   \
+        else if (ne == 2) WG_LAUNCH_RO(D3, 2, E8_);                                                              \
+        else if (ne == 3) WG_LAUNCH_RO(D3, 3, E8_);                                                              \
+        else if (ne == 4) WG_LAUNCH_RO(D3, 4, E8_);                                                              \
+        else WG_LAUNCH_RO(D3, 8, E8_);                                                                           \
     } while (0)
-    if (in3d) WG_RO_NE(true); else WG_RO_NE(false);
+    if (in3d) { if (e8) WG_RO_NE(true, true); else WG_RO_NE(true, false); }
+    else { if (e8) WG_RO_NE(false, true); else WG_RO_NE(false, false); }
 #undef WG_RO_NE
 #undef WG_LAUNCH_RO
     const hipError_t e = hipGetLastError();
@@ -2784,7 +2825,8 @@
 
 int run(const wg_batch *b, const wg_params *p, const float *action, int32_t cols, int32_t astride,
         int64_t astep, const wg_outputs *o, int32_t n_steps, const int32_t *plan, int32_t plan_blocks,
-        hipStream_t stream, bool step, bool resident = false, bool check_only = false, int s_first = 0) {
+        hipStream_t stream, bool step, bool resident = false, bool check_only = false, int s_first = 0,
+        int s_total = 0) {
     int rc = validate(b);
     if (rc) return rc;
     if (!p) return fail(WG_EINVAL, "null params");
@@ -2796,7 +2838,7 @@
     if (b->ragged && (!plan || plan_blocks <= 0)) return fail(WG_EINVAL, "ragged batch needs a plan");
     wg_outputs out = o ? *o : wg_outputs{};
     if (out.obs && out.obs_stride <= 0) return fail(WG_EINVAL, "obs_stride must be > 0");
-    const KParams kp = make_kparams(*p);
+    KParams kp = make_kparams(*p);
     const Geo g = b->ragged ? ragged_geo(b) : uniform_geo(b, out.obs ? out.obs_stride : 0, step && p->pair_mode != 0);
     if (g.W > g.threads) return fail(WG_ERANGE, "more than %d walkers per workgroup", g.threads);
     const int blocks = b->ragged ? plan_blocks : (b->N + g.W - 1) / g.W;
@@ -2827,7 +2869,9 @@
     if (resident && use_lean && p->pair_mode == 0 && !extras)
         return launch_lean_rollout(b, kp, p->in3d != 0, action, cols, astride, action ? astep : 0, out, n_steps, lg,
                                    stream);
+    const int s_last = (s_total > 0 ? s_total : s_first + n_steps) - 1;
     for (int s = s_first; s < s_first + n_steps; s++) {
+        kp.keep_aux = (s_total < 0 || s >= s_last || extras) ? 1 : 0;
         wg_outputs os = out;
         if (os.obs) os.obs += s * os.obs_step;
         if (os.reward) os.reward += s * os.out_step;
@@ -2898,7 +2942,7 @@
     auto issue = [&](int i, int s) -> int {
         const wg_range &r = ranges[i];
         return run(r.batch, p, action ? action + r.action_offset : nullptr, action_cols, action_stride, action_step,
-                   r.outputs, 1, r.plan, r.plan_blocks, r.stream, true, false, false, s);
+                   r.outputs, 1, r.plan, r.plan_blocks, r.stream, true, false, false, s, n_steps);
     };
     int rc = 0;
     for (int s = 0; s < n_steps && !rc; s++)
@@ -2955,7 +2999,7 @@
     for (int s = 0; s < n_steps && !rc; s++) {
         g_kev_start = ev[2 * s]; g_kev_stop = ev[2 * s + 1];
         rc = run(b, p, action, action_cols, action_stride, action_step, o, 1, plan, plan_blocks, stream, true, false,
-                 false, s);
+                 false, s, -1);
     }
     g_kev_start = g_kev_stop = nullptr;
     double total = 0.0;
diff --git a/walker_gym_amd/device.py b/walker_gym_amd/device.py
--- a/walker_gym_amd/device.py
+++ b/walker_gym_amd/device.py
@@ -8,7 +8,7 @@
 import torch
 
 from . import _lib
-from .layout import HostLayout, default_radius
+from .layout import HostLayout, default_radius, refresh_edges8, set_springs
 
 
 def _to_dev(a: np.ndarray, device) -> torch.Tensor:
@@ -46,6 +46,9 @@
         self.acc = _to_dev(host.acc, dv)
         self.mass = _to_dev(host.mass, dv)
         self.edges = _to_dev(host.edges, dv)
+        if host.edges8 is None:
+            refresh_edges8(host)
+        self._upload_edges8()
         self.inc = _to_dev(host.inc, dv) if host.E else None
         self.inc_off = _to_dev(host.inc_off, dv)
         self.muscle_x = _to_dev(host.muscle_x, dv)
@@ -72,6 +75,25 @@
         self.version = 0
         self.replan(wave_ok)
 
+    def _upload_edges8(self) -> None:
+        host = self.host
+        if host.edges8 is None:
+            self.edges8, self.kc = None, (0.0, 0.0, 0.0, 0.0)
+        else:
+            self.edges8, self.kc = _to_dev(host.edges8, self.device), tuple(float(x) for x in host.kc)
+
+    def set_springs(self, ei=None, ej=None, rest=None, k=None, c=None, flags=None) -> None:
+        topo = set_springs(self.host, ei=ei, ej=ej, rest=rest, k=k, c=c, flags=flags)
+        if self.E:
+            self.edges.copy_(_to_dev(self.host.edges, self.device))
+        if topo:
+            if self.inc is not None:
+                self.inc.copy_(_to_dev(self.host.inc, self.device))
+            self.inc_off.copy_(_to_dev(self.host.inc_off, self.device))
+        self._upload_edges8()
+        self.version += 1
+        self.struct = self._make_struct()
+
     def replan(self, wave_ok: bool) -> None:
         host, L = self.host, _lib.load()
         self.wave_ok = bool(wave_ok)
@@ -140,7 +162,8 @@
             muscle_x=self._p(self.muscle_x), muscle_bounds=self._p(self.muscle_bounds),
             muscle_stride=self._p(self.muscle_stride), steps=self._p(self.steps), contact=self._p(self.contact),
             pinned=self._p(self.pinned), charge=self._p(self.charge), radius=self._p(self.radius),
-            bounce_set=self._p(self.bounce_set))
+            bounce_set=self._p(self.bounce_set),
+            edges8=self._p(self.edges8) if not r else None, kc=(C.c_float * 4)(*self.kc))
 
     def sub_struct(self, w0: int, w1: int) -> _lib.WgBatch:
         if self.ragged:
@@ -163,7 +186,9 @@
             muscle_stride=self._p(self.muscle_stride) if A == 0 else off(self.muscle_stride, A * w0),
             steps=off(self.steps, w0), contact=off(self.contact, M * w0), pinned=off(self.pinned, M * w0),
             charge=off(self.charge, M * w0), radius=off(self.radius, M * w0), row=None,
-            bounce_set=off(self.bounce_set, M * w0))
+            bounce_set=off(self.bounce_set, M * w0),
+            edges8=off(self.edges8, 2 * K * w0) if self.edges8 is not None and w0 % (64 // M) == 0 else None,
+            kc=(C.c_float * 4)(*self.kc))
 
     def launch_geometry(self) -> dict:
         info = _lib.WgLaunchInfo()
diff --git a/walker_gym_amd/layout.py b/walker_gym_amd/layout.py
--- a/walker_gym_amd/layout.py
+++ b/walker_gym_amd/layout.py
@@ -40,6 +40,8 @@
     row: Optional[np.ndarray] = None
     mass_perm: Optional[np.ndarray] = None
     muscle_perm: Optional[np.ndarray] = None
+    edges8: Optional[np.ndarray] = None
+    kc: Optional[np.ndarray] = None
     extra: Dict[str, np.ndarray] = field(default_factory=dict)
 
     @property
@@ -116,6 +118,7 @@
             row, mass_perm, muscle_perm = order.astype(np.int32), spec["_mass_perm"], spec["_muscle_perm"]
     lay = _pack(spec, spec.get("mx"), spec.get("steps"))
     lay.row, lay.mass_perm, lay.muscle_perm = row, mass_perm, muscle_perm
+    refresh_edges8(lay)
     return lay
 
 
@@ -175,6 +178,91 @@
     )
 
 
+EDGE8_MUSCLE = np.uint32(1 << 30)
+EDGE8_STRING = np.uint32(1 << 31)
+
+
+def edge8_classes(edges: np.ndarray, K: int, A: int):
+    edges = np.asarray(edges, np.uint32).reshape(-1, 4)
+    mus = (np.arange(len(edges)) % max(K, 1)) < A
+    out = []
+    for sel in (mus, ~mus):
+        kc = edges[sel][:, 2:4]
+        if len(kc) == 0:
+            out.append(None)
+            continue
+        if np.any(kc != kc[0]):
+            return None
+        out.append((int(kc[0, 0]), int(kc[0, 1])))
+    if out[0] is None and out[1] is None:
+        out = [(0, 0), (0, 0)]
+    m, o = (out[0] or out[1]), (out[1] or out[0])
+    return np.array([m[0], m[1], o[0], o[1]], np.uint32)
+
+
+def pack_edges8(lay: "HostLayout"):
+    M, K, A = lay.M, lay.K, lay.A
+    if lay.ragged or M < 4 or M > 64 or 64 % M or K < 1 or lay.E == 0:
+        return None
+    wpw = 64 // M
+    if wpw * A > 64:
+        return None
+    kc = edge8_classes(lay.edges, K, A)
+    if kc is None:
+        return None
+    e = np.arange(lay.E, dtype=np.int64)
+    wt, k = (e // K) % wpw, e % K
+    ij = lay.edges[:, 0].astype(np.int64)
+    i, j = ij & 0x7fff, (ij >> 16) & 0x7fff
+    mus = k < A
+    w = ((wt * M + i) * 4) | (((wt * M + j) * 4) << 8) | (np.where(mus, (wt * A + k) * 4, 0) << 16)
+    w = w.astype(np.uint32) | np.where(mus, EDGE8_MUSCLE, np.uint32(0)) | (lay.edges[:, 0] & EDGE8_STRING)
+    return np.ascontiguousarray(np.stack([w, lay.edges[:, 1]], axis=1), np.uint32), kc.view(f32).copy()
+
+
+def refresh_edges8(lay: "HostLayout") -> None:
+    packed = pack_edges8(lay)
+    lay.edges8, lay.kc = (None, None) if packed is None else packed
+
+
+def set_springs(lay: "HostLayout", ei=None, ej=None, rest=None, k=None, c=None, flags=None) -> bool:
+    E = lay.E
+    ed = np.asarray(lay.edges, np.uint32).reshape(-1, 4).copy()
+
+    def full(v, dtype):
+        return np.ascontiguousarray(np.broadcast_to(np.asarray(v, dtype), (E,)))
+
+    topo = ei is not None or ej is not None
+    if topo or flags is not None:
+        i = (ed[:, 0] & np.uint32(0x7fff)) if ei is None else full(ei, np.int64).astype(np.uint32)
+        j = ((ed[:, 0] >> np.uint32(16)) & np.uint32(0x7fff)) if ej is None else full(ej, np.int64).astype(np.uint32)
+        st = (ed[:, 0] >> np.uint32(31)) if flags is None else (full(flags, np.uint8) & 1).astype(np.uint32)
+        if topo:
+            lay.inc, lay.inc_off = incidence(i.astype(np.int64), j.astype(np.int64), lay.mass_off, lay.edge_off)
+        ed[:, 0] = i | (j << np.uint32(16)) | (st << np.uint32(31))
+    for col, v in ((1, rest), (2, k), (3, c)):
+        if v is not None:
+            ed[:, col] = full(v, f32).view(np.uint32)
+    lay.edges = np.ascontiguousarray(ed, np.uint32)
+    refresh_edges8(lay)
+    return topo
+
+
+def unpack_edges8(edges8: np.ndarray, M: int, K: int, A: int) -> Dict[str, np.ndarray]:
+    w = np.asarray(edges8, np.uint32).reshape(-1, 2)[:, 0].astype(np.int64)
+    bi, bj, xoff = w & 0xff, (w >> 8) & 0xff, (w >> 16) & 0xff
+    return dict(bi=bi, bj=bj, xoff=xoff, wt=(bi >> 2) // M, ei=(bi >> 2) % M, ej=(bj >> 2) % M,
+                rest=np.asarray(edges8, np.uint32).reshape(-1, 2)[:, 1].copy().view(f32),
+                muscle=((w >> 30) & 1).astype(bool), string=((w >> 31) & 1).astype(bool))
+
+
+def compact_bytes_per_walker_step(M, K, A, obs_floats, info: bool = True, contact: bool = True, last: bool = False):
+    b = layout_bytes_per_walker_step(M, K, A, obs_floats, info=info, contact=contact) - 8 * K
+    if not last:
+        b = b - 12 * M - (M if contact else 0)
+    return b
+
+
 def _per_mass_f64(spec, key: str, P: int):
     a = spec.get(key)
     if a is None:
```

Result: faster. 2.110 billion (median of 6 runs) (+5.2%).
